# soedinglab/MMseqs2

Measured on AMD Instinct MI355X. Metric: sw_gcells_per_s, higher is better.
Workload: dtype int16

## Files before the change

mmseqs2_amd/csrc/mmgpu_internal.h:

```cpp
#ifndef MMGPU_INTERNAL_H
#define MMGPU_INTERNAL_H

#include <hip/hip_runtime.h>
#include <stdint.h>
#include <cstdlib>
#include <cstring>

#include <algorithm>
#include <array>
#include <string>
#include <map>
#include <mutex>
#include <chrono>
#include <memory>
#include <vector>
#include <thread>
#include <atomic>

#include "../../include/mmgpu.h"
#include "nucl_core.h"
#include "block_plan.h"

namespace mmgpu {

struct DeviceDb {
    uint8_t *res = nullptr;
    uint32_t *off4 = nullptr;
    uint32_t *len = nullptr;
    uint32_t n = 0;
    uint32_t max_len = 0;
    uint64_t total_residues = 0;
    int alphabet = 0;
    size_t res_bytes = 0;
};

struct TargetView {
    const uint8_t *res = nullptr;
    const uint32_t *off4 = nullptr;
    const uint32_t *len = nullptr;
    uint32_t n = 0;
    uint32_t max_len = 0;
    const uint32_t *h_len = nullptr;
};

struct SwMaskGatherArgs {
    const uint8_t *src_res;
    const uint32_t *src_off4, *src_len;
    const uint32_t *src_id;
    uint8_t *dst_res;
    const uint32_t *dst_off4;
    const uint32_t *span_off;
    const mmgpu_sw_span *spans;
    uint32_t span_base;
    uint32_t mask_letter;
    uint32_t n_pairs;
};
hipError_t launch_sw_mask_gather(const SwMaskGatherArgs &A, hipStream_t stream);

struct SwJob {
    uint32_t query;
    uint32_t hit_begin;
    uint32_t hit_end;
    uint32_t shape;
};

struct SwLaunch {
    const SwJob *jobs;
    uint32_t n_jobs;
    const uint8_t *q_res;
    const int8_t *q_cb;
    const uint32_t *q_off;
    const int32_t *q_bias;
    const int32_t *q_minstart;
    const int8_t *q_prof;
    const uint32_t *q_prof_off;
    const uint8_t *t_res;
    const uint32_t *t_off4;
    const uint32_t *t_len;
    const uint32_t *hit_target;
    const uint32_t *hit_out;
    mmgpu_sw_hit *out;
    const int8_t *mat;
    int alphabet;
    int gap_open, gap_extend;
    uint2 *scratch;
    uint32_t scratch_cols;
    uint32_t *scratch_busy;
    uint32_t scratch_slots;
    uint32_t resident_lds = 0;
    const uint32_t *q_hit_count;
    uint32_t hit_stride;
    int rev_mode = 0;
    int rev_only = 0;
    const uint8_t *rev_force = nullptr;
};

constexpr int SW_PF_MAX_LIST = 16384;
constexpr int SW_FROM_PF_STAT_SLOTS = 64;

struct SwFromPfArgs {
    const mmgpu_pf_hit *pf_hits;
    uint32_t pf_stride;
    const uint32_t *hit_count;
    uint32_t stride;
    const uint32_t *q_off;
    const uint32_t *t_len;
    uint32_t *hit_target, *hit_out;
    unsigned long long *cells, *pairs;
    uint32_t *count_copy;
    uint32_t *slot_target;
};

constexpr int SW_REV_JOB_MAX = 1024;
hipError_t launch_sw_rev_multi(const SwLaunch &L, size_t lds_bytes, hipStream_t stream);
hipError_t launch_sw_from_pf(const SwFromPfArgs &A, uint32_t nq, hipStream_t stream);
uint32_t sw_multi_resident_blocks(size_t lds_bytes, bool both_passes, int compute_units);

#ifndef MMGPU_SW_MAX_R
#define MMGPU_SW_MAX_R 28
#endif
constexpr int SW_MAX_R = MMGPU_SW_MAX_R;
static_assert(SW_MAX_R >= 16 && SW_MAX_R <= 32, "multi-tile bodies exist for 8..32 rows per lane: a query cut into tiles gets at least SW_MAX_R / 2");
#ifndef MMGPU_SW_MIN_WAVES
#define MMGPU_SW_MIN_WAVES 2
#endif
constexpr int SW_MIN_WAVES = MMGPU_SW_MIN_WAVES;
#ifndef MMGPU_SW_GROUPS
#define MMGPU_SW_GROUPS 4
#endif
constexpr int SW_GROUPS = MMGPU_SW_GROUPS;
static_assert(SW_GROUPS == 3 || SW_GROUPS == 4, "three or four kernel groups");
int sw_shape_group(uint32_t shape);
hipError_t launch_sw(const SwLaunch &L, int group, size_t lds_bytes, bool both_passes, hipStream_t stream);

constexpr int SW_LDS_HEADER = SW_REV_JOB_MAX * 2 + 64;
__host__ __device__ constexpr int lane_stride_bytes(int R) {
    int slots = (R * 2 + 15) / 16;
    if ((slots & 1) == 0) slots += 1;
    return slots * 16;
}
__host__ __device__ constexpr uint32_t sw_profile_bytes(int R, int alphabet) {
    return (uint32_t)(alphabet + 1) * 16u * (uint32_t)lane_stride_bytes(R);
}
#ifndef MMGPU_SW_RESIDENT_LDS
#define MMGPU_SW_RESIDENT_LDS 65536
#endif
constexpr uint32_t SW_RESIDENT_LDS = MMGPU_SW_RESIDENT_LDS;
static_assert(SW_RESIDENT_LDS <= 65536u, "a workgroup asks for at most 64 KB of dynamic LDS");
__host__ __device__ constexpr uint32_t sw_tiles(uint32_t qlen, int R) { return (qlen + 16u * (uint32_t)R - 1u) / (16u * (uint32_t)R); }
__host__ __device__ constexpr bool sw_multi_resident(uint32_t n_tiles, int R, int alphabet, uint32_t budget) {
    return (unsigned long long)n_tiles * sw_profile_bytes(R, alphabet) + (unsigned long long)SW_LDS_HEADER <= (unsigned long long)budget;
}
static_assert(sw_multi_resident(2, 28, 21, 65536) && sw_multi_resident(3, 24, 21, 65536) && !sw_multi_resident(3, 25, 21, 65536) &&
              !sw_multi_resident(4, 22, 21, 65536) && !sw_multi_resident(2, 8, 21, 0), "residency rule");

constexpr int SCAN_CLASSES = 5;
constexpr int SCAN_MULTI = SCAN_CLASSES - 1;
constexpr int SCAN_MAX_R = 32;
constexpr int SCAN_ROUND = 32;
constexpr int SCAN_JOB_TARGETS = 16 * SCAN_ROUND;
constexpr int SCAN_MAX_HITS = 4096;
__host__ __device__ constexpr int scan_class_rows(int cls) { return cls == 0 ? 8 : cls == 1 ? 16 : cls == 2 ? 24 : 32; }
__host__ __device__ constexpr uint32_t scan_cols(uint32_t len, int R) { return (len + (uint32_t)R - 1u) / (uint32_t)R * (uint32_t)R; }
__host__ __device__ constexpr uint32_t scan_park_row_words(uint32_t longest) { return 2u * ((scan_cols(longest, SCAN_MAX_R) + 1u + 15u) & ~15u); }

constexpr uint64_t SCAN_NO_PROFILE = ~0ull;

struct ScanJob {
    uint32_t query;
    uint32_t begin, end;
    uint32_t pad;
};

struct ScanLaunch {
    const ScanJob *jobs;
    uint32_t n_jobs;
    const uint8_t *q_res;
    const int8_t *q_cb;
    const uint32_t *q_off;
    const int32_t *q_cap;
    const int8_t *q_prof;
    const uint64_t *q_prof_off;
    const uint32_t *q_prof_letters;
    const uint8_t *t_res;
    const uint32_t *t_off4, *t_len;
    const uint32_t *order;
    uint32_t n_targets;
    const int8_t *mat;
    int alphabet;
    uint8_t *scores;
    uint32_t *park;
    const uint64_t *park_off;
};
hipError_t launch_scan(const ScanLaunch &L, int cls, uint32_t grid, hipStream_t stream);

struct ScanSelectArgs {
    const uint8_t *scores;
    const uint32_t *t_len;
    uint32_t n_targets;
    const uint32_t *q_ident;
    const uint32_t *q_win;
    int32_t min_score;
    uint32_t max_hits;
    mmgpu_pf_hit *hits;
    uint32_t stride;
    uint32_t *counts;
};
hipError_t launch_scan_select(const ScanSelectArgs &A, uint32_t nq, hipStream_t stream);
void warm_scan();

constexpr int PF_T = 4096;
constexpr int PF_IDS_PER_BIN = 4096;
constexpr int PF_SAT_CAP = 1024;
constexpr int PF_CAND0 = 32;
constexpr int PF_QSTAGE = 2048;
constexpr int PF_MAX_HITS = 4096;
constexpr int PF_MAX_HITS_BIG = 131072;

struct PfList {
    uint32_t start;
    uint32_t len;
    uint32_t lprefix;
    uint32_t pos;
};

struct PfCand {
    uint32_t id;
    uint32_t arr;
    uint32_t score;
    uint16_t diag;
    uint16_t pad;
};

__host__ __device__ inline uint32_t pf_el_count(uint32_t s) { return (s & 0x80000000u) ? ((s >> 23) & 0xFFu) : (s < 255u ? s : 255u); }
__host__ __device__ inline uint32_t pf_el_exact(uint32_t s) { return (s & 0x80000000u) ? (s & 0x7FFFFFu) : s; }

constexpr int PF_PROW = 32;
constexpr int PF_PROF_LETTERS = 20;

struct PfKmerArgs {
    const uint8_t *q_res;
    const int16_t *q_thr;
    uint32_t n_pos;
    uint8_t pat[16];
    uint32_t kalph, n3;
    uint32_t kbase;
    const int16_t *s3;
    const uint32_t *i3;
    const uint32_t *offsets;
    const uint32_t *nonempty;
    const uint4 *cofs;
    const uint16_t *cum3;
    uint32_t cum_w;
    int32_t score_min;
    int k;
    const int16_t *s2;
    const uint32_t *i2;
    const uint16_t *cum2;
    uint32_t cum2_w;
    int32_t score2_min;
    const uint8_t *q_kind;
    const int16_t *prof_score;
    const uint8_t *prof_letter;
    int exact;
    const uint32_t *order;
    uint32_t *nsim;
    const uint32_t *list_base;
    PfList *lists;
    uint32_t *pos_entries;
};

struct PfSplitArgs {
    const uint32_t *tile_q, *tile_idx;
    const uint32_t *q_off;
    const uint32_t *q_entries;
    const uint32_t *pos_entry_base;
    const uint32_t *list_base;
    const PfList *lists;
    const uint64_t *idx_entries;
    uint32_t bins;
    uint32_t *split;
    uint8_t *split_hi;
    uint16_t *bin_off;
    uint32_t *bucket_count;
};

struct PfDedupArgs {
    uint32_t n_queries, bins;
    uint32_t q_first;
    uint32_t cand_origin;
    const uint32_t *q_tile_base, *q_ntiles;
    const uint32_t *split;
    const uint8_t *split_hi;
    const uint16_t *bin_off;
    const uint32_t *cand_base;
    PfCand *cand, *surv;
    PfCand *cand_small;
    uint32_t *surv_count;
    uint32_t *cand_count;
    uint64_t *cell_counter;
    const uint32_t *q_off;
    const uint8_t *q_res;
    const int8_t *q_corr;
    const int8_t *mat;
    int alphabet;
    const int8_t *q_rows;
    const uint8_t *q_isprof;
    int nucl;
    uint32_t sort_cap;
    uint32_t *q_ncand;
    PfCand *sat;
    uint32_t *q_nsat;
    uint32_t sat_cap;
    const uint8_t *t_res;
    const uint32_t *t_off4, *t_len;
    uint32_t min_diag_score;
    uint32_t *q_flags;
    uint32_t ref_bins;
    uint32_t *big_list, *big_count;
    const uint32_t *q_nseg;
    const uint32_t *seg_start;
};

struct PfSelectArgs {
    uint32_t q_first, cand_origin;
    int kmer_score;
    const PfCand *surv;
    const uint32_t *cand_base;
    uint32_t bins;
    const uint32_t *surv_count;
    const uint32_t *q_identity;
    const int32_t *q_self_score;
    uint32_t max_hits, min_diag_score, ref_bins;
    mmgpu_pf_hit *hits;
    uint32_t hit_stride;
    uint32_t *hit_count, *q_diag_thr;
    mmgpu_pf_xhit *xhits;
    const uint32_t *global_ids;
    const uint32_t *q_nseg;
    uint32_t *q_flags;
    const uint32_t *cand_count;
    uint32_t cand_cap;
    int nucl;
    uint64_t *big_keys;
    uint16_t *big_diags;
    uint32_t big_stride;
    const uint32_t *q_off, *peb, *list_base;
    const PfList *lists;
};

constexpr int PF_XMERGE_CAP = 4096;
struct PfXMergeArgs {
    const mmgpu_pf_xhit *xhits;
    const uint32_t *counts;
    uint32_t n_shards, nq, stride;
    uint32_t max_hits, min_diag_score, ref_bins;
    const int32_t *q_self_score;
    const uint32_t *q_identity;
    mmgpu_pf_hit *out_hits;
    uint32_t out_stride;
    uint32_t *out_counts;
    uint32_t *out_flags;
};
hipError_t launch_pf_xmerge(const PfXMergeArgs &A, hipStream_t s);

struct PfLocalizeArgs {
    const mmgpu_pf_hit *hits;
    const uint32_t *counts;
    uint32_t nq, stride, shard;
    const uint32_t *shard_of, *local_id;
    mmgpu_pf_hit *local_hits;
    uint32_t *local_counts;
    uint32_t *local_slot;
};
hipError_t launch_pf_localize(const PfLocalizeArgs &A, hipStream_t s);

struct SwOwnedRec {
    mmgpu_sw_hit hit;
    uint32_t slot;
    uint32_t pad;
};
struct SwOwnedPackArgs {
    const mmgpu_sw_hit *res;
    const uint32_t *local_counts;
    const uint32_t *local_slot;
    uint32_t nq, stride;
    SwOwnedRec *send;
    uint32_t cap;
    uint32_t *counter;
};
struct SwOwnedScatterArgs {
    const SwOwnedRec *recv;
    const uint32_t *counters;
    uint32_t n_ranks, cap, n_slots;
    mmgpu_sw_hit *full;
    uint32_t *status;
};
hipError_t launch_sw_owned_pack(const SwOwnedPackArgs &A, hipStream_t s);
hipError_t launch_sw_owned_scatter(const SwOwnedScatterArgs &A, hipStream_t s);

constexpr int PF_MAX_SEG = 62;

struct PfSegArgs {
    const uint32_t *ovf_queries;
    uint32_t n_ovf;
    const uint32_t *q_off, *list_base, *pos_entry_base;
    const PfList *lists;
    uint64_t cap;
    uint32_t *seg_start;
    uint32_t *q_nseg;
    uint32_t *q_final;
    const uint32_t *q_entries;
};

struct PfOvfElem {
    uint32_t id;
    uint32_t score;
    long long ord;
    uint16_t diag;
    uint16_t pad0;
    uint32_t pad1;
};

struct PfOvfArgs {
    PfDedupArgs D;
    const uint32_t *ovf_queries;
    uint32_t n_ovf;
    uint32_t step;
    const uint32_t *q_final;
    const uint64_t *ovf_base;
    PfOvfElem *buf_a, *buf_b;
    uint32_t *o_count;
    uint32_t *totals;
};

hipError_t launch_pf_segments(const PfSegArgs &A, hipStream_t s);
hipError_t launch_pf_overflow(const PfOvfArgs &A, hipStream_t s);

constexpr int PF_MERGE_CAP = 8192;

struct PfMergeArgs {
    const mmgpu_pf_hit *hits;
    const uint32_t *counts;
    uint32_t n_splits, nq, stride;
    uint32_t id_offset[64];
    mmgpu_pf_hit *out_hits;
    uint32_t *out_counts;
};

hipError_t launch_pf_merge(const PfMergeArgs &A, hipStream_t s);
hipError_t launch_pf_kmers(const PfKmerArgs &A, bool emit, hipStream_t s);
size_t pf_cofs_bytes(uint64_t table);
hipError_t launch_pf_cofs(const uint32_t *offsets, uint64_t table, void *cofs, hipStream_t s);
hipError_t db_section_checksum(const void *dev, size_t bytes, unsigned long long *scratch, uint64_t *sum, hipStream_t s);
hipError_t db_validate_layout(const uint32_t *off4, const uint32_t *len, uint32_t n, uint64_t res_bytes, uint32_t max_len, const uint32_t *offsets,
                              uint64_t table, const uint64_t *entries, uint64_t n_entries, uint32_t *scratch, uint32_t *bad, hipStream_t s);
hipError_t launch_pf_tiles(const uint32_t *q_tile_base, const uint32_t *q_ntiles, uint32_t nq, uint32_t *tile_q, uint32_t *tile_idx, hipStream_t s);
hipError_t launch_pf_bitmap(const uint32_t *offsets, uint64_t table, uint32_t *bitmap, unsigned long long *nonempty, hipStream_t s);
hipError_t launch_pf_scan(const uint32_t *in, const uint32_t *q_off, uint32_t nq, const uint64_t *base, uint32_t *out,
                          uint64_t *totals, hipStream_t s);
hipError_t launch_pf_split(const PfSplitArgs &A, uint32_t n_tiles, hipStream_t s);
hipError_t launch_pf_dedup(const PfDedupArgs &A, hipEvent_t after_replay, hipEvent_t after_ungapped, hipStream_t s);
hipError_t launch_pf_count(const PfDedupArgs &A, hipEvent_t after_a, hipEvent_t after_b, hipStream_t s);
hipError_t launch_pf_long(const PfDedupArgs &A, bool long_queries, hipStream_t s);
hipError_t launch_pf_select(const PfSelectArgs &A, uint32_t nq, hipStream_t s);

struct IxArgs {
    const uint8_t *t_res;
    const uint32_t *t_off4, *t_len;
    uint32_t n_targets;
    int k, pattern_len, kmer_thr;
    uint32_t kalph;
    uint8_t pat[16];
    int8_t self_score[32];
    uint32_t *counts;
    const uint32_t *offsets;
    uint64_t *entries;
    uint32_t *scratch;
};

struct IxSortArgs {
    uint64_t table;
    const uint32_t *offsets;
    const uint64_t *src;
    uint64_t *dst;
    uint32_t *long_lists;
    uint32_t *n_long;
    uint32_t long_cap;
};

hipError_t launch_ix_target(const IxArgs &A, bool fill, hipStream_t s);

struct TantanArgs {
    const uint8_t *t_res;
    uint8_t *out_res;
    const uint32_t *t_off4, *t_len;
    const uint32_t *order;
    uint32_t n;
    const double *lr;
    const double *b2f;
    int alphabet;
    double repeat_prob, repeat_end_prob, min_mask_prob;
    uint8_t mask_letter;
    float *probs;
    double *scales;
    const uint64_t *wave_prob_base, *wave_scale_base;
    unsigned long long *n_masked;
};
hipError_t launch_tantan_mask(const TantanArgs &A, hipStream_t s);
void warm_sw();
void warm_block();
void warm_pf();
void warm_ix();
void warm_tantan();
void warm_bt();
hipError_t launch_ix_sort_short(const IxSortArgs &A, hipStream_t s);
hipError_t launch_ix_sort_long(const IxSortArgs &A, uint32_t n_long, hipStream_t s);

struct BtJob {
    uint32_t slot;
    uint32_t query, target;
    int32_t q_start, q_end, t_start, t_end, score;
    uint64_t bt_off;
};

struct BtLaunch {
    const BtJob *jobs;
    uint32_t n_jobs;
    const uint8_t *q_res;
    const int8_t *q_cb;
    const uint32_t *q_off;
    const int8_t *q_prof;
    const uint32_t *q_prof_off;
    const uint8_t *t_res;
    const uint32_t *t_off4;
    const int8_t *mat;
    int alphabet, gap_open, gap_extend;
    uint32_t *scratch;
    uint32_t words_per_lane;
    uint32_t band_cap;
    mmgpu_sw_bt *info;
    char *bt;
    uint8_t *dir_pool;
    unsigned long long dir_pool_bytes;
    unsigned long long *dir_cursor;
};

struct BlockLaunch {
    const BlockJob *jobs;
    uint32_t n_jobs;
    const uint8_t *q_res;
    const int8_t *q_cb;
    const uint32_t *q_off;
    const uint8_t *t_res;
    const uint32_t *t_off4;
    const int8_t *q_prof;
    const uint32_t *q_prof_off;
    int alphabet;
    const int8_t *scores;
    int gap_open, gap_extend;
    mmgpu_sw_block *out;
    const uint64_t *bt_off;
    char *bt;
    uint8_t *pool;
    uint64_t slot_bytes;
    uint32_t n_pool_slots;
    uint32_t *pool_busy;
    uint32_t *growth = nullptr;
    uint32_t growth_cap = 0;
};
hipError_t launch_sw_block(const BlockLaunch &L, int tier, hipStream_t stream);

struct Block2Launch {
    const Block2Job *jobs;
    uint32_t n_jobs;
    uint32_t *counter;
    const uint8_t *q_res;
    const int8_t *q_cb;
    const uint32_t *q_off;
    const uint8_t *t_res;
    const uint32_t *t_off4;
    const int8_t *scores;
    int gap_open, gap_extend;
    mmgpu_sw_block *out;
    const uint64_t *bt_off;
    char *bt;
    uint8_t *pool;
    uint32_t *growth = nullptr;
    uint32_t growth_cap = 0;
    uint8_t *ck_pool = nullptr;
    uint32_t trace_bytes = 0;
};
constexpr int BLOCK4_MAX_SIZE = 128;
constexpr int BLOCK4_LARGE_SIZE = 256;
constexpr int BLOCK4_SKEW_SIZE = 1024;
hipError_t launch_sw_block4(const Block2Launch &L, bool trace, int form, uint32_t n_waves, hipStream_t stream);
hipError_t launch_sw_block4_walk(const Block2Launch &L, hipStream_t stream);
void warm_block4();

struct BlockSelectArgs {
    const mmgpu_sw_hit *res;
    uint32_t pairs;
    const uint32_t *qout_off;
    uint32_t n_queries;
    const int32_t *q_minstart;
    const uint32_t *slot_target;
    BlockJob *jobs;
    uint32_t *pair_of_slot;
    mmgpu_sw_block *blk;
    uint32_t *count;
    uint32_t cap;
};
struct BlockScatterArgs {
    const mmgpu_sw_block *blk;
    const uint32_t *pair_of_slot;
    uint32_t n;
    mmgpu_sw_hit *res;
    uint8_t *rev_force;
    uint32_t *counts;
};
hipError_t launch_block_select(const BlockSelectArgs &A, hipStream_t stream);
hipError_t launch_block_scatter(const BlockScatterArgs &A, hipStream_t stream);

hipError_t launch_sw_traceback(const BtLaunch &L, hipStream_t stream);
hipError_t launch_sw_traceback_wave(const BtLaunch &L, hipStream_t stream);

inline unsigned host_threads() {
    unsigned n = std::thread::hardware_concurrency();
    return n == 0 ? 1 : std::min(n, 64u);
}

template <typename F>
inline void parallel_for(size_t n, F f) {
    const unsigned nt = (unsigned)std::min<size_t>(host_threads(), std::max<size_t>(n, 1));
    if (nt <= 1 || n < 4096) {
        f((size_t)0, n);
        return;
    }
    std::vector<std::thread> th;
    const size_t chunk = (n + nt - 1) / nt;
    for (unsigned t = 0; t < nt; t++) {
        const size_t a = std::min(n, (size_t)t * chunk), b = std::min(n, a + chunk);
        if (a < b) th.emplace_back([=] { f(a, b); });
    }
    for (auto &x : th) x.join();
}

extern thread_local std::string g_last_error;
inline int fail(int code, const std::string &msg) {
    g_last_error = msg;
    return code;
}
#define HIP_TRY(expr)                                                                                      \
    do {                                                                                                   \
        hipError_t e__ = (expr);                                                                           \
        if (e__ != hipSuccess)                                                                             \
            return mmgpu::fail(MMGPU_ERR_HIP, std::string(#expr) + ": " + hipGetErrorString(e__));         \
    } while (0)

inline hipError_t dev_malloc(void **p, size_t n) { return hipMalloc(p, n); }
inline void dev_free(void *p) {
    if (p) (void)hipFree(p);
}

struct BlockCache {
    std::multimap<size_t, void *> blocks;
    size_t cached = 0;
    bool closed = false;
    std::mutex lock;
    static size_t limit() {
        static const size_t v = []() -> size_t {
            size_t f = 0, t = 0;
            if (hipMemGetInfo(&f, &t) != hipSuccess || t == 0) return (size_t)16 << 30;
            return t / 3;
        }();
        return v;
    }
    static size_t round_up(size_t n) {
        if (n <= 512) return 512;
        int top = 63 - __builtin_clzll((unsigned long long)n);
        const size_t step = (size_t)1 << (top - 2);
        return (n + step - 1) & ~(step - 1);
    }
    void *take(size_t &cap) {
        std::lock_guard<std::mutex> guard(lock);
        auto it = blocks.lower_bound(cap);
        if (it == blocks.end() || it->first > 2 * cap) return nullptr;
        void *p = it->second;
        cap = it->first;
        blocks.erase(it);
        cached -= cap;
        return p;
    }
    void give(void *p, size_t cap) {
        std::lock_guard<std::mutex> guard(lock);
        if (closed || cached + cap > limit()) { dev_free(p); return; }
        blocks.emplace(cap, p);
        cached += cap;
    }
    void trim() {
        std::lock_guard<std::mutex> guard(lock);
        for (auto &kv : blocks) dev_free(kv.second);
        blocks.clear();
        cached = 0;
    }
};

struct DevBuf {
    void *p = nullptr;
    size_t bytes = 0;
    size_t cap = 0;
    std::shared_ptr<BlockCache> cache;
    DevBuf() = default;
    DevBuf(const DevBuf &) = delete;
    DevBuf &operator=(const DevBuf &) = delete;
    DevBuf(DevBuf &&o) noexcept : p(o.p), bytes(o.bytes), cap(o.cap), cache(std::move(o.cache)) { o.p = nullptr; o.bytes = 0; o.cap = 0; }
    DevBuf &operator=(DevBuf &&o) noexcept {
        if (this != &o) {
            release();
            p = o.p; bytes = o.bytes; cap = o.cap; cache = std::move(o.cache);
            o.p = nullptr; o.bytes = 0; o.cap = 0;
        }
        return *this;
    }
    ~DevBuf() { release(); }
    void bind(const std::shared_ptr<BlockCache> &c) {
        cache = c;
    }
    void release() {
        if (!p) return;
        if (cache && cap) cache->give(p, cap);
        else dev_free(p);
        p = nullptr;
        cap = 0;
    }
    hipError_t alloc(size_t n) {
        release();
        bytes = n;
        if (n == 0) return hipSuccess;
        if (cache) {
            cap = BlockCache::round_up(n);
            p = cache->take(cap);
            if (p) return hipSuccess;
            hipError_t e = dev_malloc(&p, cap);
            if (e != hipSuccess) {
                (void)hipGetLastError();
                cache->trim();
                e = dev_malloc(&p, cap);
            }
            if (e != hipSuccess) { p = nullptr; cap = 0; bytes = 0; }
            return e;
        }
        const hipError_t e = dev_malloc(&p, n);
        if (e != hipSuccess) { p = nullptr; bytes = 0; (void)hipGetLastError(); }
        return e;
    }
    hipError_t reserve(size_t n) { return n <= bytes ? hipSuccess : alloc(n + n / 8); }
    template <typename T> T *as() const { return reinterpret_cast<T *>(p); }
};

struct SideStream {
    hipStream_t s = nullptr;
    SideStream() = default;
    SideStream(const SideStream &) = delete;
    SideStream &operator=(const SideStream &) = delete;
    ~SideStream() { if (s) { (void)hipStreamSynchronize(s); (void)hipStreamDestroy(s); } }
    hipError_t create() { return s ? hipSuccess : hipStreamCreateWithFlags(&s, hipStreamNonBlocking); }
};

struct PinnedStage {
    uint8_t *p = nullptr;
    hipEvent_t moved = nullptr;
    PinnedStage() = default;
    PinnedStage(const PinnedStage &) = delete;
    PinnedStage &operator=(const PinnedStage &) = delete;
    ~PinnedStage() { if (p) (void)hipHostFree(p); if (moved) (void)hipEventDestroy(moved); }
    hipError_t reserve(size_t bytes, bool with_event = true) {
        const hipError_t e = hipHostMalloc((void **)&p, bytes, hipHostMallocDefault);
        if (e != hipSuccess) { p = nullptr; return e; }
        return with_event ? hipEventCreateWithFlags(&moved, hipEventDisableTiming) : hipSuccess;
    }
};

struct UploadRing {
    SideStream up;
    std::vector<PinnedStage> slots;
    UploadRing() = default;
    UploadRing(const UploadRing &) = delete;
    UploadRing &operator=(const UploadRing &) = delete;
    ~UploadRing() { if (up.s) (void)hipStreamSynchronize(up.s); }
    hipError_t open(size_t n_slots) { slots = std::vector<PinnedStage>(n_slots); return up.create(); }
    hipError_t wait(size_t k) const { return hipEventSynchronize(slots[k].moved); }
    hipError_t sent(size_t k) const { return hipEventRecord(slots[k].moved, up.s); }
};

struct DbBuild {
    DeviceDb db;
    uint8_t *masked = nullptr;
    DbBuild() = default;
    DbBuild(const DbBuild &) = delete;
    DbBuild &operator=(const DbBuild &) = delete;
    ~DbBuild() { dev_free(db.res); dev_free(db.off4); dev_free(db.len); dev_free(masked); }
    DeviceDb take_db() { DeviceDb d = db; db = DeviceDb(); return d; }
    uint8_t *take_masked() { uint8_t *m = masked; masked = nullptr; return m; }
};

template <typename T>
inline hipError_t upload(DevBuf &b, const std::vector<T> &v, hipStream_t s) {
    hipError_t e = b.alloc(std::max<size_t>(v.size(), 1) * sizeof(T));
    if (e != hipSuccess) return e;
    if (v.empty()) return hipSuccess;
    return hipMemcpyAsync(b.p, v.data(), v.size() * sizeof(T), hipMemcpyHostToDevice, s);
}

inline size_t upload_pinned_need(size_t bytes) { return (bytes + 255) & ~(size_t)255; }
template <typename T>
inline hipError_t upload_pinned(DevBuf &b, const std::vector<T> &v, hipStream_t s, void *base, size_t cap, size_t &used) {
    hipError_t e = b.alloc(std::max<size_t>(v.size(), 1) * sizeof(T));
    if (e != hipSuccess) return e;
    if (v.empty()) return hipSuccess;
    const size_t n = v.size() * sizeof(T);
    if (!base || used + upload_pinned_need(n) > cap) return hipMemcpyAsync(b.p, v.data(), n, hipMemcpyHostToDevice, s);
    void *st = static_cast<char *>(base) + used;
    used += upload_pinned_need(n);
    memcpy(st, v.data(), n);
    return hipMemcpyAsync(b.p, st, n, hipMemcpyHostToDevice, s);
}

hipError_t launch_nucl_align(const NuclLaunch &L, unsigned blocks, hipStream_t stream);
hipError_t launch_nucl_align_wave(const NuclLaunch &L, unsigned blocks, hipStream_t stream);

hipError_t launch_pf_order(const PfKmerArgs &A, uint32_t *order, const std::shared_ptr<BlockCache> &cache, hipStream_t s);

struct PfIndex;

}

namespace mmgpu {
struct Comm {
    void *nccl = nullptr;
    int rank = 0, n_ranks = 1;
    std::string transport;
};
}

struct mmgpu_ctx {
    int device = 0;
    mmgpu::Comm *comm = nullptr;
    hipStream_t stream = nullptr;
    bool owns_stream = false;
    mmgpu::DeviceDb db;
    std::vector<uint32_t> h_len;
    uint32_t mean_len = 0;
    int compute_units = 0;
    std::string name;
    mmgpu::PfIndex *pf = nullptr;
    uint8_t *pf_masked_res = nullptr;
    const uint8_t *pf_res() const { return pf_masked_res ? pf_masked_res : db.res; }
    struct Shard {
        bool on = false;
        uint32_t n_shards = 1, shard = 0, global_n = 0;
        mmgpu::DevBuf d_global_ids, d_shard_of, d_local_id;
    } shard;
    std::shared_ptr<mmgpu::BlockCache> cache = std::make_shared<mmgpu::BlockCache>();
    hipStream_t side[4] = {};
    hipEvent_t fork = nullptr, join[4] = {};
    void *pinned = nullptr;
    size_t pinned_cap = 0;
    std::atomic<bool> pinned_busy{false};
    mmgpu::DevBuf scan_scores, scan_park;
    uint64_t scan_serial = 0;
};

inline hipError_t dev_malloc_ctx(mmgpu_ctx *c, void **p, size_t n) {
    hipError_t e = mmgpu::dev_malloc(p, n);
    if (e != hipSuccess && c && c->cache) {
        (void)hipGetLastError();
        c->cache->trim();
        e = mmgpu::dev_malloc(p, n);
    }
    return e;
}

struct mmgpu_pf_batch_t;
struct mmgpu_sw_batch_t;
namespace mmgpu {
int comm_require_rccl();
int comm_group_start();
int comm_group_end();
int comm_init_all(mmgpu_ctx **ctxs, int n);
int comm_allgather(mmgpu_ctx *c, const void *send, void *recv, size_t bytes);
void comm_free(mmgpu_ctx *c);
struct XchgBlock { const void *send; void *recv; size_t bytes; };
int pf_xchg_begin(mmgpu_ctx *c, mmgpu_pf_batch_t *b, int n_ranks, XchgBlock blocks[2]);
int pf_xchg_merge(mmgpu_ctx *c, mmgpu_pf_batch_t *b, int n_ranks, const uint32_t *identity_global);
struct PfRedoRows {
    std::vector<uint32_t> q;
    std::vector<mmgpu_pf_hit> hits;
    std::vector<uint32_t> counts;
    std::vector<int32_t> status;
    uint32_t stride = 0;
};
int pf_redo_flagged(mmgpu_ctx *c, mmgpu_pf_batch_t *b, std::vector<uint32_t> &flagged);
int pf_redo_run(mmgpu_ctx *full, const mmgpu_pf_params *par, const mmgpu_pf_query *qs, const std::vector<uint32_t> &flagged, PfRedoRows &rows);
int pf_redo_apply(mmgpu_ctx *c, mmgpu_pf_batch_t *b, const PfRedoRows &rows);
const int32_t *pf_batch_redo_status(const mmgpu_pf_batch_t *b);
int sw_gather_begin(mmgpu_ctx *c, mmgpu_sw_batch_t *b, int n_ranks, XchgBlock blocks[2]);
int sw_gather_finish(mmgpu_ctx *c, mmgpu_sw_batch_t *b, int n_ranks);
int sw_gather_overflowed(mmgpu_ctx *c, mmgpu_sw_batch_t *b, bool *overflowed);
int pf_batch_merged_flags(mmgpu_pf_batch_t *b, const void **d_flags);
const int32_t *pf_batch_host_status(const mmgpu_pf_batch_t *b);
bool pf_batch_merged_lists(mmgpu_pf_batch_t *b, const mmgpu_pf_hit **hits, const uint32_t **counts, uint32_t *stride, uint32_t *nq);
void pf_index_free(mmgpu_ctx *c);
void db_release(mmgpu_ctx *c);
bool pf_batch_device_lists(mmgpu_pf_batch_t *b, const mmgpu_pf_hit **hits, const uint32_t **counts, uint32_t *stride, uint32_t *nq);
}
#endif
```

mmseqs2_amd/csrc/sw_kernel.hip:

```cpp
#include "mmgpu_internal.h"
#include "pf_device.h"

namespace mmgpu {

namespace {

constexpr int GROUP = 16;
constexpr int WAVES = 4;
constexpr int GROUPS_PER_WAVE = 64 / GROUP;
constexpr int HITS_PER_WAVE = 2 * GROUPS_PER_WAVE;
constexpr unsigned NEG2 = 0x80008000u;

typedef short s16x2 __attribute__((ext_vector_type(2)));
typedef unsigned short u16x2 __attribute__((ext_vector_type(2)));

__device__ __forceinline__ unsigned pk_add_sat(unsigned a, unsigned b) {
    return __builtin_bit_cast(unsigned, __builtin_elementwise_add_sat(__builtin_bit_cast(s16x2, a),
                                                                      __builtin_bit_cast(s16x2, b)));
}
__device__ __forceinline__ unsigned pk_max_s(unsigned a, unsigned b) {
    return __builtin_bit_cast(unsigned, __builtin_elementwise_max(__builtin_bit_cast(s16x2, a),
                                                                  __builtin_bit_cast(s16x2, b)));
}
__device__ __forceinline__ unsigned pk_max_u(unsigned a, unsigned b) {
    return __builtin_bit_cast(unsigned, __builtin_elementwise_max(__builtin_bit_cast(u16x2, a),
                                                                  __builtin_bit_cast(u16x2, b)));
}
__device__ __forceinline__ unsigned pk_sub_sat_u(unsigned a, unsigned b) {
    return __builtin_bit_cast(unsigned, __builtin_elementwise_sub_sat(__builtin_bit_cast(u16x2, a),
                                                                      __builtin_bit_cast(u16x2, b)));
}
__device__ __forceinline__ unsigned bfi(unsigned mask, unsigned a, unsigned b) {
    return (a & mask) | (b & ~mask);
}
__device__ __forceinline__ unsigned from_lane_above(unsigned head, unsigned v) {
    return __builtin_amdgcn_update_dpp(head, v, 0x111 , 0xF, 0xF, false);
}
__device__ __forceinline__ unsigned from_lane_above_or_zero(unsigned v) {
    return __builtin_amdgcn_update_dpp(0u, v, 0x111 , 0xF, 0xF, true);
}

#ifndef MMGPU_SW_PREFETCH
#define MMGPU_SW_PREFETCH 1
#endif
#define SW_KEEP_IN_ROW(x) asm volatile("" : "+v"(x))

template <int R>
struct Tile {
    static constexpr int ROWS = GROUP * R;
    static constexpr int LANE_STRIDE = lane_stride_bytes(R);
    static constexpr int ROW_STRIDE = GROUP * LANE_STRIDE;
};
static_assert(GROUP == 16, "sw_profile_bytes and sw_tiles (mmgpu_internal.h) assume 16-lane groups");

template <int R, bool REV>
__device__ __forceinline__ void build_profile(unsigned char *lds, const uint8_t *q, const int8_t *cb, int qlen,
                                              int tile_base, const int8_t *mat, int alphabet, const int8_t *prof) {
    using T = Tile<R>;
    const int total = (alphabet + 1) * T::ROWS;
    for (int idx = threadIdx.x; idx < total; idx += blockDim.x) {
        const int letter = idx / T::ROWS;
        const int row = idx - letter * T::ROWS;
        const int rg = tile_base + row;
        short v = (short)-32768;
        if (letter < alphabet && rg < qlen) {
            const int qi = REV ? (qlen - 1 - rg) : rg;
            v = prof ? (short)prof[letter * qlen + qi] : (short)((int)mat[letter * alphabet + q[qi]] + (int)cb[qi]);
        }
        const int lane = row / R, r = row - lane * R;
        *reinterpret_cast<short *>(lds + letter * T::ROW_STRIDE + lane * T::LANE_STRIDE + r * 2) = v;
    }
}

__device__ __forceinline__ bool sw_rev_wanted(const SwLaunch &L, uint32_t slot, int min_start) {
    const mmgpu_sw_hit &f = L.out[slot];
    const int s = f.score;
    if (L.rev_mode == 2) return s > 0 && L.rev_force[slot] != 0;
    return s > 0 && s >= min_start && !(L.rev_mode == 1 && f.word != 0);
}

constexpr int SW_REV_JOB_HITS = 1024;
static_assert(SW_REV_JOB_HITS == SW_REV_JOB_MAX, "host and kernel disagree on the reverse job size");
static_assert(SW_LDS_HEADER == SW_REV_JOB_HITS * 2 + 64, "the header holds the live hits and the scheduling words");

template <int R, bool MULTI, bool REV, bool PF>
__device__ __forceinline__ void sw_body(const SwLaunch &L, const SwJob job) {
    using T = Tile<R>;
    extern __shared__ __attribute__((aligned(16))) unsigned char lds_all[];
    uint16_t *live = reinterpret_cast<uint16_t *>(lds_all);
    uint32_t *live_wave = reinterpret_cast<uint32_t *>(lds_all + SW_REV_JOB_HITS * 2);
    uint32_t *next_chunk = reinterpret_cast<uint32_t *>(lds_all + SW_REV_JOB_HITS * 2 + 16);
    unsigned char *lds = lds_all + SW_LDS_HEADER;
    if (MULTI) __builtin_amdgcn_s_setprio(3);
    const int lane = threadIdx.x & 63;
    const int wave = __builtin_amdgcn_readfirstlane(threadIdx.x >> 6);
    const int g = lane & (GROUP - 1);
    const int grp = lane / GROUP;

    const uint32_t qbeg = L.q_off[job.query];
    const int qlen = (int)(L.q_off[job.query + 1] - qbeg);
    const uint8_t *q = L.q_res + qbeg;
    const int8_t *cb = L.q_cb + qbeg;
    const int qbias = L.q_bias[job.query];
    const int8_t *prof = nullptr;
    if (L.q_prof_off) {
        const uint32_t po = L.q_prof_off[job.query];
        if (po != 0xFFFFFFFFu) prof = L.q_prof + po;
    }
    const int n_tiles = MULTI ? (int)sw_tiles((uint32_t)qlen, R) : 1;
    const uint32_t tile_bytes = sw_profile_bytes(R, L.alphabet);
    const bool resident = MULTI && sw_multi_resident((uint32_t)n_tiles, R, L.alphabet, L.resident_lds);
    const bool dynamic = !MULTI || resident;
    auto build_all_tiles = [&]() {
        for (int tile = 0; tile < n_tiles; ++tile)
            build_profile<R, REV>(lds + (uint32_t)tile * tile_bytes, q, cb, qlen, tile * T::ROWS, L.mat, L.alphabet, prof);
        __syncthreads();
    };

    const unsigned go2 = (unsigned)L.gap_open * 0x10001u;
    const unsigned ge2 = (unsigned)L.gap_extend * 0x10001u;
    const unsigned pad_letter = (unsigned)L.alphabet;

    if (threadIdx.x == 0) *next_chunk = 0;
    if (!MULTI && !REV) {
        build_profile<R, REV>(lds, q, cb, qlen, 0, L.mat, L.alphabet, prof);
        __syncthreads();
    }
    if (MULTI && !REV && resident) build_all_tiles();

    uint32_t n_hits = job.hit_end - job.hit_begin;
    if (REV) {
        const int min_start = L.q_minstart[job.query];
        uint32_t total = 0;
        for (uint32_t base = 0; base < n_hits; base += WAVES * 64) {
            const uint32_t idx = base + threadIdx.x;
            bool pass = false;
            if (idx < n_hits) pass = sw_rev_wanted(L, L.hit_out[job.hit_begin + idx], min_start);
            const unsigned long long bal = __ballot(pass);
            if (lane == 0) live_wave[wave] = (uint32_t)__popcll(bal);
            __syncthreads();
            uint32_t before = 0, round_total = 0;
#pragma unroll
            for (int w = 0; w < WAVES; ++w) {
                const uint32_t c = live_wave[w];
                before += w < wave ? c : 0u;
                round_total += c;
            }
            if (pass) live[total + before + (uint32_t)__popcll(bal & ((1ull << lane) - 1ull))] = (uint16_t)idx;
            total += round_total;
            __syncthreads();
        }
        n_hits = total;
        if (n_hits == 0) return;
        if (!MULTI) {
            build_profile<R, REV>(lds, q, cb, qlen, 0, L.mat, L.alphabet, prof);
            __syncthreads();
        }
        if (MULTI && resident) build_all_tiles();
    }
    const uint32_t n_iter = (n_hits + WAVES * HITS_PER_WAVE - 1) / (WAVES * HITS_PER_WAVE);

    for (uint32_t it = 0; dynamic || it < n_iter; ++it) {
        uint32_t chunk = it * WAVES + wave;
        if (dynamic) {
            if (lane == 0) chunk = atomicAdd(next_chunk, 1u);
            chunk = __builtin_amdgcn_readfirstlane(chunk);
        }
        const uint32_t slot0 = chunk * HITS_PER_WAVE;
        if (dynamic && slot0 >= n_hits) break;

        const uint32_t sA = slot0 + grp * 2, sB = sA + 1;
        const bool vA = sA < n_hits, vB = sB < n_hits;
        const uint32_t hA = job.hit_begin + (REV ? (uint32_t)live[vA ? sA : 0] : sA);
        const uint32_t hB = job.hit_begin + (REV ? (uint32_t)live[vB ? sB : 0] : sB);
        const uint32_t tA = vA ? L.hit_target[hA] : 0u, tB = vB ? L.hit_target[hB] : 0u;
        const uint8_t *pA = L.t_res + (size_t)L.t_off4[tA] * 4;
        const uint8_t *pB = L.t_res + (size_t)L.t_off4[tB] * 4;
        int colsA = vA ? (int)L.t_len[tA] : 0, colsB = vB ? (int)L.t_len[tB] : 0;
        int r0A = 0, r0B = 0;
        int endA = 0, endB = 0;
        unsigned rev_target = 0xFFFFFFFFu;
        if (REV) {
            mmgpu_sw_hit fa, fb;
            fa.score = 0; fa.q_end = 0; fa.t_end = 0;
            fb = fa;
            if (vA) fa = L.out[L.hit_out[hA]];
            if (vB) fb = L.out[L.hit_out[hB]];
            colsA = vA ? fa.t_end + 1 : 0;
            colsB = vB ? fb.t_end + 1 : 0;
            endA = colsA > 0 ? fa.t_end : 0;
            endB = colsB > 0 ? fb.t_end : 0;
            r0A = colsA > 0 ? qlen - 1 - fa.q_end : 0;
            r0B = colsB > 0 ? qlen - 1 - fb.q_end : 0;
            rev_target = (colsA > 0 ? (unsigned)fa.score & 0xFFFFu : 0xFFFFu) | ((colsB > 0 ? (unsigned)fb.score & 0xFFFFu : 0xFFFFu) << 16);
        }
        int ncols = colsA > colsB ? colsA : colsB;
        ncols = max(ncols, __shfl_xor(ncols, 16));
        ncols = max(ncols, __shfl_xor(ncols, 32));
        ncols = __builtin_amdgcn_readfirstlane(ncols);
        const int nsteps = ncols + GROUP - 1;
        int mincols = colsA < colsB ? colsA : colsB;
        mincols = min(mincols, __shfl_xor(mincols, 16));
        mincols = min(mincols, __shfl_xor(mincols, 32));
        mincols = __builtin_amdgcn_readfirstlane(mincols);

        unsigned long long bestA = 0, bestB = 0;

        uint2 *scr = nullptr;
        unsigned scr_grp = 0;
        if (MULTI) {
            scr = L.scratch + (size_t)((job.shape >> 8) * WAVES + wave) * GROUPS_PER_WAVE * 2 * L.scratch_cols;
            scr_grp = (unsigned)grp * 2u * L.scratch_cols;
        }

        for (int tile = 0; tile < n_tiles; ++tile) {
            const int tile_base = tile * T::ROWS;
            if (MULTI && !resident) {
                __syncthreads();
                build_profile<R, REV>(lds, q, cb, qlen, tile_base, L.mat, L.alphabet, prof);
                __syncthreads();
            }
            const unsigned char *const lds_tile = MULTI && resident ? lds + (uint32_t)tile * tile_bytes : lds;
            const uint2 *scr_in = MULTI ? scr + (size_t)((tile + 1) & 1) * L.scratch_cols : nullptr;
            uint2 *scr_out = MULTI ? scr + (size_t)(tile & 1) * L.scratch_cols : nullptr;
            const bool has_above = MULTI && tile > 0;
            const bool has_below = MULTI && tile + 1 < n_tiles;

            unsigned Hp[R], E[R], aux[R];
#pragma unroll
            for (int r = 0; r < R; ++r) { Hp[r] = 0; E[r] = 0; aux[r] = 0; }
            if (REV) {
#pragma unroll
                for (int r = 0; r < R; ++r) {
                    const int rg = tile_base + g * R + r;
                    aux[r] = (rg >= r0A ? 0xFFFFu : 0u) | (rg >= r0B ? 0xFFFF0000u : 0u);
                }
            }
            unsigned vmax = 0, bestcol = 0xFFFFFFFFu;
            unsigned rev_rowA = 0, rev_rowB = 0;
            unsigned Hup_prev = 0;
            unsigned out_H = 0, out_F = 0;

            auto letters4 = [&](const uint8_t *p, int end, int k) -> unsigned {
                if (!REV) return reinterpret_cast<const unsigned *>(p)[k];
                int o = end - 3 - 4 * k;
                o = o < -3 ? -3 : o;
                unsigned w;
                __builtin_memcpy(&w, p + o, 4);
                return w;
            };
            unsigned wA = letters4(pA, endA, 0), wB = letters4(pB, endB, 0);
            unsigned wA_next = letters4(pA, endA, 1), wB_next = letters4(pB, endB, 1);
            uint2 bnd = make_uint2(0, 0), bnd_next = make_uint2(0, 0);
            auto boundary16 = [&](int m) -> uint2 {
                const int last = ncols - 1 < 0 ? 0 : ncols - 1;
                return scr_in[scr_grp + (unsigned)min(16 * m + g - (m > 0 ? 1 : 0), last)];
            };
            if (has_above) {
                bnd = boundary16(0);
                bnd_next = boundary16(1);
            }

            constexpr int ND = (R + 1) / 2;
            unsigned pav_next[PF ? ND : 1], pbv_next[PF ? ND : 1];
            auto load_rows = [&](unsigned letters, unsigned *pav, unsigned *pbv) {
                const unsigned a = letters & 0xFFu, b = (letters >> 8) & 0xFFu;
                const uint4 *rowA = reinterpret_cast<const uint4 *>(lds_tile + a * T::ROW_STRIDE + g * T::LANE_STRIDE);
                const uint4 *rowB = reinterpret_cast<const uint4 *>(lds_tile + b * T::ROW_STRIDE + g * T::LANE_STRIDE);
#pragma unroll
                for (int k = 0; k < ND / 4; ++k) {
                    const uint4 pa = rowA[k], pb = rowB[k];
                    pav[4 * k] = pa.x; pav[4 * k + 1] = pa.y; pav[4 * k + 2] = pa.z; pav[4 * k + 3] = pa.w;
                    pbv[4 * k] = pb.x; pbv[4 * k + 1] = pb.y; pbv[4 * k + 2] = pb.z; pbv[4 * k + 3] = pb.w;
                }
                if constexpr (ND % 4 >= 2) {
                    const uint2 pa = *reinterpret_cast<const uint2 *>(rowA + ND / 4);
                    const uint2 pb = *reinterpret_cast<const uint2 *>(rowB + ND / 4);
                    pav[(ND / 4) * 4] = pa.x; pav[(ND / 4) * 4 + 1] = pa.y;
                    pbv[(ND / 4) * 4] = pb.x; pbv[(ND / 4) * 4 + 1] = pb.y;
                }
                if constexpr (ND % 2 == 1) {
                    pav[ND - 1] = reinterpret_cast<const unsigned *>(rowA)[ND - 1];
                    pbv[ND - 1] = reinterpret_cast<const unsigned *>(rowB)[ND - 1];
                }
            };
            unsigned let = pad_letter * 0x101u;
            constexpr bool LETTER_BLOCKS = MULTI || REV || R >= 7;
            constexpr bool LETTER_QUEUE = !MULTI && R < 7;
            unsigned long long lq = 0;
            auto letter_block = [&](int k) {
                if (!LETTER_BLOCKS) return;
                unsigned a = wA, b = wB;
                if (4 * k + 4 > mincols) {
                    const unsigned pad4 = pad_letter * 0x01010101u;
                    const int na = min(max(colsA - 4 * k, 0), 4), nb = min(max(colsB - 4 * k, 0), 4);
                    const unsigned ma = REV ? ~(unsigned)(0xFFFFFFFFull >> (8 * na)) : (unsigned)((1ull << (8 * na)) - 1ull);
                    const unsigned mb = REV ? ~(unsigned)(0xFFFFFFFFull >> (8 * nb)) : (unsigned)((1ull << (8 * nb)) - 1ull);
                    a = bfi(ma, a, pad4);
                    b = bfi(mb, b, pad4);
                }
                const unsigned lo = __builtin_amdgcn_perm(b, a, REV ? 0x06020703u : 0x05010400u);
                const unsigned hi = __builtin_amdgcn_perm(b, a, REV ? 0x04000501u : 0x07030602u);
                lq = ((unsigned long long)hi << 32) | lo;
            };
            auto head_letters = [&](int c, int j) -> unsigned {
                if (LETTER_BLOCKS && LETTER_QUEUE) { const unsigned v = (unsigned)lq; lq >>= 16; return v; }
                if (LETTER_BLOCKS) return (unsigned)(lq >> (16 * j));
                const unsigned sh = (unsigned)(REV ? 3 - j : j) * 8u;
                const unsigned la0 = __builtin_amdgcn_ubfe(wA, sh, 8u);
                const unsigned lb0 = __builtin_amdgcn_ubfe(wB, sh, 8u);
                return (c < colsA ? la0 : pad_letter) | ((c < colsB ? lb0 : pad_letter) << 8);
            };
            letter_block(0);
            let = from_lane_above(head_letters(0, 0), let);
            if (PF) load_rows(let, pav_next, pbv_next);

            for (int s0 = -1; s0 < nsteps; s0 += 4) {
            if (MULTI && s0 > 0 && ((s0 + 1) & 15) == 0) {
                bnd = bnd_next;
                if (has_above) bnd_next = boundary16(((s0 + 1) >> 4) + 1);
            }
            const int jn = min(4, nsteps - s0);
#pragma nounroll
            for (int j = s0 < 0 ? 1 : 0; j < jn; ++j) {
                const int s = s0 + j;
                if (has_below && s >= GROUP) {
                    if (g == GROUP - 1) (scr_out + (s - GROUP))[scr_grp] = make_uint2(out_H, out_F);
                }
                const unsigned Hup = MULTI ? from_lane_above(bnd.x, out_H) : from_lane_above_or_zero(out_H);
                unsigned f = MULTI ? from_lane_above(bnd.y, out_F) : from_lane_above_or_zero(out_F);
                if (MULTI) {
                    bnd.x = __builtin_amdgcn_update_dpp(bnd.x, bnd.x, 0x12F, 0xF, 0xF, false);
                    bnd.y = __builtin_amdgcn_update_dpp(bnd.y, bnd.y, 0x12F, 0xF, 0xF, false);
                }
                unsigned pav[ND], pbv[ND];
                if (PF) {
#pragma unroll
                    for (int k = 0; k < ND; ++k) { pav[k] = pav_next[k]; pbv[k] = pbv_next[k]; }
                } else {
                    load_rows(let, pav, pbv);
                }

                unsigned hd = Hup_prev;
                Hup_prev = Hup;
                unsigned cmax = 0;
                unsigned pre[R], es[R];
#pragma unroll
                for (int r = 0; r < R; ++r) {
                    unsigned P = __builtin_amdgcn_perm(pbv[r / 2], pav[r / 2], (r & 1) ? 0x07060302u : 0x05040100u);
                    if (REV) P = __builtin_amdgcn_bitop3_b32(aux[r], P, NEG2, 0xCA);
                    pre[r] = pk_max_s(pk_add_sat(r == 0 ? hd : Hp[r - 1], P), E[r]);
                    es[r] = pk_sub_sat_u(E[r], ge2);
                }
                let = from_lane_above(head_letters(s + 1, j), let);
                if (PF) load_rows(let, pav_next, pbv_next);
#pragma unroll
                for (int r = 0; r < R; ++r) {
                    const unsigned h = pk_max_s(pre[r], f);
                    const unsigned fs = pk_sub_sat_u(f, ge2);
                    const unsigned t = pk_sub_sat_u(h, go2);
                    cmax = pk_max_u(cmax, h);
                    f = pk_max_u(fs, t);
                    E[r] = pk_max_u(es[r], t);
                    SW_KEEP_IN_ROW(E[r]);
                    Hp[r] = h;
                }
                out_H = Hp[R - 1];
                out_F = f;

                const int col = s - g;

                const unsigned nm = pk_max_u(vmax, cmax);
                if (nm != vmax) {
                    const unsigned diff = nm ^ vmax;
                    if (!REV) {
                        const unsigned mask = ((diff & 0xFFFFu) ? 0xFFFFu : 0u) | ((diff >> 16) ? 0xFFFF0000u : 0u);
                        bestcol = bfi(mask, ((unsigned)col & 0xFFFFu) * 0x10001u, bestcol);
#pragma unroll
                        for (int r = 0; r < R; ++r) aux[r] = bfi(mask, Hp[r], aux[r]);
                    } else {
                        const unsigned x = nm ^ rev_target;
                        const bool hitA = (diff & 0xFFFFu) && !(x & 0xFFFFu), hitB = (diff >> 16) && !(x >> 16);
                        if (hitA | hitB) {
                            asm volatile("" ::: "memory");
                            unsigned ra = 0, rb = 0;
#pragma unroll
                            for (int r = R - 1; r >= 0; --r) {
                                if ((Hp[r] & 0xFFFFu) == (rev_target & 0xFFFFu)) ra = (unsigned)r;
                                if ((Hp[r] >> 16) == (rev_target >> 16)) rb = (unsigned)r;
                            }
                            if (hitA) { bestcol = (bestcol & 0xFFFF0000u) | ((unsigned)col & 0xFFFFu); rev_rowA = ra; }
                            if (hitB) { bestcol = (bestcol & 0xFFFFu) | ((unsigned)col << 16); rev_rowB = rb; }
                        }
                    }
                    vmax = nm;
                }
            }
            {
                wA = wA_next; wB = wB_next;
                const int k = ((s0 + 1) >> 2) + 2;
                wA_next = letters4(pA, endA, k); wB_next = letters4(pB, endB, k);
                letter_block(k - 1);
            }
            }
            if (has_below && ncols > 0 && g == GROUP - 1) (scr_out + (ncols - 1))[scr_grp] = make_uint2(out_H, out_F);

            unsigned rowA_first = rev_rowA, rowB_first = rev_rowB;
            unsigned sA = vmax & 0xFFFFu, sB = vmax >> 16;
            if (!REV) {
#pragma unroll
                for (int r = R - 1; r >= 0; --r) {
                    if ((aux[r] & 0xFFFFu) == sA) rowA_first = (unsigned)r;
                    if ((aux[r] >> 16) == sB) rowB_first = (unsigned)r;
                }
            } else {
                sA = sA == (rev_target & 0xFFFFu) ? sA : 0u;
                sB = sB == (rev_target >> 16) ? sB : 0u;
            }
            const unsigned rgA = (unsigned)(tile_base + g * R) + rowA_first;
            const unsigned rgB = (unsigned)(tile_base + g * R) + rowB_first;
            unsigned long long keyA = sA ? ((unsigned long long)sA << 32) | ((0xFFFFu - (bestcol & 0xFFFFu)) << 16) | (0xFFFFu - rgA) : 0ull;
            unsigned long long keyB = sB ? ((unsigned long long)sB << 32) | ((0xFFFFu - (bestcol >> 16)) << 16) | (0xFFFFu - rgB) : 0ull;
#pragma unroll
            for (int m = 1; m < GROUP; m <<= 1) {
                const unsigned long long oa = __shfl_xor(keyA, m), ob = __shfl_xor(keyB, m);
                keyA = oa > keyA ? oa : keyA;
                keyB = ob > keyB ? ob : keyB;
            }
            bestA = keyA > bestA ? keyA : bestA;
            bestB = keyB > bestB ? keyB : bestB;
        }

        if (g == 0) {
#pragma unroll
            for (int half = 0; half < 2; ++half) {
                const bool valid = half ? vB : vA;
                if (!valid) continue;
                const unsigned long long key = half ? bestB : bestA;
                const uint32_t h = half ? hB : hA;
                const int score = (int)(key >> 32);
                const int col = 0xFFFF - (int)((key >> 16) & 0xFFFFu);
                const int row = 0xFFFF - (int)(key & 0xFFFFu);
                mmgpu_sw_hit *o = L.out + L.hit_out[h];
                if (!REV) {
                    mmgpu_sw_hit res;
                    res.score = score;
                    res.q_end = score ? row : 0;
                    res.t_end = score ? col : -1;
                    res.q_start = -1;
                    res.t_start = -1;
                    res.word = (score + qbias >= 255) ? 1 : 0;
                    *o = res;
                } else {
                    const int end = half ? endB : endA;
                    const int cols = half ? colsB : colsA;
                    if (cols > 0) {
                        o->t_start = (score == o->score) ? end - col : -2;
                        o->q_start = (score == o->score) ? qlen - 1 - row : -2;
                    }
                }
            }
        }
    }
}

template <int R, bool MULTI, bool BOTH>
__device__ __forceinline__ void sw_passes(const SwLaunch &L, const SwJob &job) {
    if constexpr (R <= SW_MAX_R) {
        constexpr bool PF = MMGPU_SW_PREFETCH && !MULTI && (BOTH || R <= 24);
        if (!(BOTH && L.rev_only)) sw_body<R, MULTI, false, PF>(L, job);
        if constexpr (BOTH && !MULTI) {
            __threadfence_block();
            __syncthreads();
            sw_body<R, MULTI, true, PF>(L, job);
        }
    }
}

#ifndef MMGPU_SW_WAVES_G0F
#define MMGPU_SW_WAVES_G0F 4
#endif
#ifndef MMGPU_SW_WAVES_G0B
#define MMGPU_SW_WAVES_G0B 2
#endif
#ifndef MMGPU_SW_WAVES_G1F
#define MMGPU_SW_WAVES_G1F 3
#endif
#ifndef MMGPU_SW_WAVES_G1B
#define MMGPU_SW_WAVES_G1B 2
#endif
#define MMGPU_SW_MULTI_ALL                                                                                                          \
    MMGPU_SW_MULTI(8) MMGPU_SW_MULTI(9) MMGPU_SW_MULTI(10) MMGPU_SW_MULTI(11) MMGPU_SW_MULTI(12) MMGPU_SW_MULTI(13) MMGPU_SW_MULTI(14) \
    MMGPU_SW_MULTI(15) MMGPU_SW_MULTI(16) MMGPU_SW_MULTI(17) MMGPU_SW_MULTI(18) MMGPU_SW_MULTI(19) MMGPU_SW_MULTI(20) MMGPU_SW_MULTI(21) \
    MMGPU_SW_MULTI(22) MMGPU_SW_MULTI(23) MMGPU_SW_MULTI(24) MMGPU_SW_MULTI(25) MMGPU_SW_MULTI(26) MMGPU_SW_MULTI(27) MMGPU_SW_MULTI(28) \
    MMGPU_SW_MULTI(29) MMGPU_SW_MULTI(30) MMGPU_SW_MULTI(31) MMGPU_SW_MULTI(32)
template <int G, bool BOTH>
__global__ __launch_bounds__(WAVES * 64)
__attribute__((amdgpu_waves_per_eu(G == 0 ? (BOTH ? MMGPU_SW_WAVES_G0B : MMGPU_SW_WAVES_G0F)
                                           : (G == 1 ? (BOTH ? MMGPU_SW_WAVES_G1B : MMGPU_SW_WAVES_G1F) : SW_MIN_WAVES),
                                   G == 1 && BOTH ? MMGPU_SW_WAVES_G1B : 8))) void sw_kernel(SwLaunch L) {
    SwJob job = L.jobs[blockIdx.x];
    if (L.q_hit_count) {
        const uint32_t lim = job.query * L.hit_stride + L.q_hit_count[job.query];
        job.hit_end = job.hit_end < lim ? job.hit_end : lim;
        if (job.hit_end <= job.hit_begin) return;
    }
    __shared__ uint32_t scratch_slot;
    const bool claims = G == SW_GROUPS - 1 && (job.shape & 0xFFu) >= 32u;
    if (claims) {
        if (threadIdx.x == 0) {
            uint32_t s = blockIdx.x % L.scratch_slots;
            while (atomicCAS(&L.scratch_busy[s], 0u, 1u) != 0u) s = s + 1 == L.scratch_slots ? 0u : s + 1;
            scratch_slot = s;
        }
        __syncthreads();
        job.shape = (job.shape & 0xFFu) | (scratch_slot << 8);
    }
#define MMGPU_SW_SINGLE(R) case (R) - 1: sw_passes<R, false, BOTH>(L, job); break;
#define MMGPU_SW_MULTI(R) case 32 + (R) - 1: sw_passes<R, true, BOTH>(L, job); break;
    if constexpr (G == 0) {
        switch (job.shape & 0xFFu) {
            MMGPU_SW_SINGLE(1) MMGPU_SW_SINGLE(2) MMGPU_SW_SINGLE(3) MMGPU_SW_SINGLE(4) MMGPU_SW_SINGLE(5) MMGPU_SW_SINGLE(6)
            MMGPU_SW_SINGLE(7) MMGPU_SW_SINGLE(8) MMGPU_SW_SINGLE(9) MMGPU_SW_SINGLE(10) MMGPU_SW_SINGLE(11) MMGPU_SW_SINGLE(12)
            default: break;
        }
    } else if constexpr (G == 1) {
        switch (job.shape & 0xFFu) {
            MMGPU_SW_SINGLE(13) MMGPU_SW_SINGLE(14) MMGPU_SW_SINGLE(15) MMGPU_SW_SINGLE(16) MMGPU_SW_SINGLE(17) MMGPU_SW_SINGLE(18)
            MMGPU_SW_SINGLE(19) MMGPU_SW_SINGLE(20) MMGPU_SW_SINGLE(21) MMGPU_SW_SINGLE(22) MMGPU_SW_SINGLE(23) MMGPU_SW_SINGLE(24)
            default: break;
        }
    } else if constexpr (SW_GROUPS == 4 && G == 2) {
        switch (job.shape & 0xFFu) {
            MMGPU_SW_SINGLE(25) MMGPU_SW_SINGLE(26) MMGPU_SW_SINGLE(27) MMGPU_SW_SINGLE(28) MMGPU_SW_SINGLE(29) MMGPU_SW_SINGLE(30)
            MMGPU_SW_SINGLE(31) MMGPU_SW_SINGLE(32)
            default: break;
        }
    } else if constexpr (SW_GROUPS == 4) {
        switch (job.shape & 0xFFu) {
            MMGPU_SW_MULTI_ALL
            default: break;
        }
    } else {
        switch (job.shape & 0xFFu) {
            MMGPU_SW_SINGLE(25) MMGPU_SW_SINGLE(26) MMGPU_SW_SINGLE(27) MMGPU_SW_SINGLE(28) MMGPU_SW_SINGLE(29) MMGPU_SW_SINGLE(30)
            MMGPU_SW_SINGLE(31) MMGPU_SW_SINGLE(32)
            MMGPU_SW_MULTI_ALL
            default: break;
        }
    }
#undef MMGPU_SW_SINGLE
#undef MMGPU_SW_MULTI
#undef MMGPU_SW_MULTI_ALL
    if (claims) {
        __syncthreads();
        if (threadIdx.x == 0) {
            __threadfence();
            atomicExch(&L.scratch_busy[scratch_slot], 0u);
        }
    }
}

__global__ __launch_bounds__(WAVES * 64) __attribute__((amdgpu_waves_per_eu(SW_MIN_WAVES))) void sw_rev_multi_kernel(SwLaunch L) {
    SwJob job = L.jobs[blockIdx.x];
    if (L.q_hit_count) {
        const uint32_t lim = job.query * L.hit_stride + L.q_hit_count[job.query];
        job.hit_end = job.hit_end < lim ? job.hit_end : lim;
        if (job.hit_end <= job.hit_begin) return;
    }
    __shared__ uint32_t scratch_slot;
    if (threadIdx.x == 0) {
        uint32_t s = blockIdx.x % L.scratch_slots;
        while (atomicCAS(&L.scratch_busy[s], 0u, 1u) != 0u) s = s + 1 == L.scratch_slots ? 0u : s + 1;
        scratch_slot = s;
    }
    __syncthreads();
    job.shape = (job.shape & 0xFFu) | (scratch_slot << 8);
#define MMGPU_SW_REV(R) case 32 + (R) - 1: if constexpr ((R) <= SW_MAX_R) sw_body<R, true, true, false>(L, job); break;
    switch (job.shape & 0xFFu) {
        MMGPU_SW_REV(8) MMGPU_SW_REV(9) MMGPU_SW_REV(10) MMGPU_SW_REV(11) MMGPU_SW_REV(12) MMGPU_SW_REV(13) MMGPU_SW_REV(14) MMGPU_SW_REV(15)
        MMGPU_SW_REV(16) MMGPU_SW_REV(17) MMGPU_SW_REV(18) MMGPU_SW_REV(19) MMGPU_SW_REV(20) MMGPU_SW_REV(21) MMGPU_SW_REV(22) MMGPU_SW_REV(23)
        MMGPU_SW_REV(24) MMGPU_SW_REV(25) MMGPU_SW_REV(26) MMGPU_SW_REV(27) MMGPU_SW_REV(28) MMGPU_SW_REV(29) MMGPU_SW_REV(30) MMGPU_SW_REV(31)
        MMGPU_SW_REV(32)
        default: break;
    }
#undef MMGPU_SW_REV
    __syncthreads();
    if (threadIdx.x == 0) {
        __threadfence();
        atomicExch(&L.scratch_busy[scratch_slot], 0u);
    }
}

__global__ __launch_bounds__(256) void sw_from_pf_kernel(SwFromPfArgs A) {
    extern __shared__ uint32_t key[];
    const uint32_t q = blockIdx.x;
    unsigned long long *const stat = A.cells + (size_t)(blockIdx.x % (uint32_t)SW_FROM_PF_STAT_SLOTS) * 3;
    const uint32_t n = min(A.hit_count[q], A.stride);
    const mmgpu_pf_hit *hits = A.pf_hits + (size_t)q * A.pf_stride;
    uint32_t np2 = 1;
    while (np2 < n) np2 <<= 1;
    unsigned long long cells = 0;
    const uint32_t qlen = A.q_off[q + 1] - A.q_off[q];
    for (uint32_t k = threadIdx.x; k < np2; k += 256) {
        uint32_t v = 0xFFFFFFFFu;
        if (k < n) {
            const uint32_t len = A.t_len[hits[k].id];
            v = ((0xFFFFu - min(len, 0xFFFFu)) << 16) | k;
            cells += (unsigned long long)qlen * len;
        }
        key[k] = v;
    }
    __syncthreads();
    const uint32_t base = q * A.stride;
    if (n <= 512) {
        for (uint32_t i = threadIdx.x; i < n; i += 256) {
            const uint32_t mine = key[i];
            uint32_t r = 0;
            for (uint32_t j = 0; j < n; j++) r += key[j] < mine ? 1u : 0u;
            A.hit_target[base + r] = hits[i].id;
            A.hit_out[base + r] = base + i;
            A.slot_target[base + i] = hits[i].id;
            if (r == 0) atomicMax(stat + 2, (unsigned long long)(0xFFFFu - (mine >> 16)));
        }
    } else {
    block_bitonic_sort<256>(np2, [&](uint32_t i, uint32_t j) { return key[i] > key[j]; }, [&](uint32_t i, uint32_t j) { exchange_at(key, i, j); });
    for (uint32_t r = threadIdx.x; r < n; r += 256) {
        const uint32_t k = key[r] & 0xFFFFu;
        A.hit_target[base + r] = hits[k].id;
        A.hit_out[base + r] = base + k;
        A.slot_target[base + r] = hits[r].id;
    }
    if (threadIdx.x == 0 && n) atomicMax(stat + 2, (unsigned long long)(0xFFFFu - (key[0] >> 16)));
    }
    for (uint32_t r = n + threadIdx.x; r < A.stride; r += 256) {
        A.hit_target[base + r] = 0;
        A.hit_out[base + r] = base + r;
        A.slot_target[base + r] = 0;
    }
    if (threadIdx.x == 0) A.count_copy[q] = n;
    wave_sum_to(stat, cells);
    if (threadIdx.x == 0 && n) atomicAdd(stat + 1, (unsigned long long)n);
}

}

hipError_t launch_sw_from_pf(const SwFromPfArgs &A, uint32_t nq, hipStream_t stream) {
    static_assert((SW_PF_MAX_LIST & (SW_PF_MAX_LIST - 1)) == 0 && (size_t)SW_PF_MAX_LIST * sizeof(uint32_t) <= 65536,
                  "SW_PF_MAX_LIST: a power of two whose dwords fit 64 KB of dynamic LDS");
    if (A.stride > (uint32_t)SW_PF_MAX_LIST) return hipErrorInvalidValue;
    if (nq == 0) return hipSuccess;
    uint32_t np2 = 1;
    while (np2 < A.stride) np2 <<= 1;
    const size_t lds = (size_t)np2 * sizeof(uint32_t);
    if (lds > 65536) return hipErrorInvalidValue;
    const hipError_t attr = hipFuncSetAttribute(reinterpret_cast<const void *>(sw_from_pf_kernel),
                                                hipFuncAttributeMaxDynamicSharedMemorySize, 65536);
    if (attr != hipSuccess) return attr;
    hipLaunchKernelGGL(sw_from_pf_kernel, dim3(nq), dim3(256), lds, stream, A);
    return hipGetLastError();
}

uint32_t sw_multi_resident_blocks(size_t lds_bytes, bool both_passes, int compute_units) {
    int per_cu = 0;
    const size_t lds = lds_bytes + SW_LDS_HEADER;
    hipError_t e = both_passes ? hipOccupancyMaxActiveBlocksPerMultiprocessor(&per_cu, sw_kernel<SW_GROUPS - 1, true>, WAVES * 64, lds)
                               : hipOccupancyMaxActiveBlocksPerMultiprocessor(&per_cu, sw_kernel<SW_GROUPS - 1, false>, WAVES * 64, lds);
    if (e == hipSuccess && both_passes) {
        int rev = 0;
        if (hipOccupancyMaxActiveBlocksPerMultiprocessor(&rev, sw_rev_multi_kernel, WAVES * 64, lds) == hipSuccess) per_cu = std::max(per_cu, rev);
    }
    if (e != hipSuccess || per_cu < 1) per_cu = 8;
    per_cu = per_cu + 1 > 8 ? 8 : per_cu + 1;
    return (uint32_t)per_cu * (uint32_t)(compute_units > 0 ? compute_units : 256);
}

hipError_t launch_sw_rev_multi(const SwLaunch &L, size_t lds_bytes, hipStream_t stream) {
    if (L.n_jobs == 0) return hipSuccess;
    hipLaunchKernelGGL(sw_rev_multi_kernel, dim3(L.n_jobs), dim3(WAVES * 64), lds_bytes + SW_LDS_HEADER, stream, L);
    return hipGetLastError();
}

int sw_shape_group(uint32_t shape) {
    if (shape >= 32) return SW_GROUPS - 1;
    const int R = (int)shape + 1;
    return R <= 12 ? 0 : (R <= 24 ? 1 : 2);
}

hipError_t launch_sw(const SwLaunch &L, int group, size_t lds_bytes, bool both_passes, hipStream_t stream) {
    static_assert(GROUP == 16, "the shape codes assume 16-lane groups");
    if (L.n_jobs == 0) return hipSuccess;
    dim3 grid(L.n_jobs), block(WAVES * 64);
    const size_t lds = lds_bytes + SW_LDS_HEADER;
    switch (group * 2 + (both_passes ? 1 : 0)) {
        case 0: hipLaunchKernelGGL((sw_kernel<0, false>), grid, block, lds, stream, L); break;
        case 1: hipLaunchKernelGGL((sw_kernel<0, true>), grid, block, lds, stream, L); break;
        case 2: hipLaunchKernelGGL((sw_kernel<1, false>), grid, block, lds, stream, L); break;
        case 3: hipLaunchKernelGGL((sw_kernel<1, true>), grid, block, lds, stream, L); break;
        case 4: hipLaunchKernelGGL((sw_kernel<2, false>), grid, block, lds, stream, L); break;
        case 5: hipLaunchKernelGGL((sw_kernel<2, true>), grid, block, lds, stream, L); break;
        case 6: hipLaunchKernelGGL((sw_kernel<SW_GROUPS - 1, false>), grid, block, lds, stream, L); break;
        case 7: hipLaunchKernelGGL((sw_kernel<SW_GROUPS - 1, true>), grid, block, lds, stream, L); break;
        default: return hipErrorInvalidValue;
    }
    return hipGetLastError();
}

void warm_sw() {
    hipFuncAttributes a;
    (void)hipFuncGetAttributes(&a, reinterpret_cast<const void *>(&sw_rev_multi_kernel));
}

}
```

Baseline: 4674.

## Add f16 packed Smith-Waterman path with int16 re-run for saturated hits

```diff
diff --git a/mmseqs2_amd/csrc/mmgpu_internal.h b/mmseqs2_amd/csrc/mmgpu_internal.h
--- a/mmseqs2_amd/csrc/mmgpu_internal.h
+++ b/mmseqs2_amd/csrc/mmgpu_internal.h
@@ -132,6 +132,11 @@
 static_assert(SW_GROUPS == 3 || SW_GROUPS == 4, "three or four kernel groups");
 int sw_shape_group(uint32_t shape);
 hipError_t launch_sw(const SwLaunch &L, int group, size_t lds_bytes, bool both_passes, hipStream_t stream);
+#ifndef MMGPU_SW_HALF
+#define MMGPU_SW_HALF 1
+#endif
+bool launch_sw_half(const SwLaunch &L, int group, size_t lds_bytes, bool both_passes, hipStream_t stream);
+void warm_sw_half();
 
 constexpr int SW_LDS_HEADER = SW_REV_JOB_MAX * 2 + 64;
 __host__ __device__ constexpr int lane_stride_bytes(int R) {
diff --git a/mmseqs2_amd/csrc/sw_body.h b/mmseqs2_amd/csrc/sw_body.h
--- /dev/null
+++ b/mmseqs2_amd/csrc/sw_body.h
@@ -0,0 +1,543 @@
+#pragma once
+#include "mmgpu_internal.h"
+#include "pf_device.h"
+
+namespace mmgpu {
+
+namespace {
+
+constexpr int GROUP = 16;
+constexpr int WAVES = 4;
+constexpr int GROUPS_PER_WAVE = 64 / GROUP;
+constexpr int HITS_PER_WAVE = 2 * GROUPS_PER_WAVE;
+constexpr unsigned NEG2 = 0x80008000u;
+
+typedef short s16x2 __attribute__((ext_vector_type(2)));
+typedef unsigned short u16x2 __attribute__((ext_vector_type(2)));
+
+__device__ __forceinline__ unsigned pk_add_sat(unsigned a, unsigned b) {
+    return __builtin_bit_cast(unsigned, __builtin_elementwise_add_sat(__builtin_bit_cast(s16x2, a),
+                                                                      __builtin_bit_cast(s16x2, b)));
+}
+__device__ __forceinline__ unsigned pk_max_s(unsigned a, unsigned b) {
+    return __builtin_bit_cast(unsigned, __builtin_elementwise_max(__builtin_bit_cast(s16x2, a),
+                                                                  __builtin_bit_cast(s16x2, b)));
+}
+__device__ __forceinline__ unsigned pk_max_u(unsigned a, unsigned b) {
+    return __builtin_bit_cast(unsigned, __builtin_elementwise_max(__builtin_bit_cast(u16x2, a),
+                                                                  __builtin_bit_cast(u16x2, b)));
+}
+__device__ __forceinline__ unsigned pk_sub_sat_u(unsigned a, unsigned b) {
+    return __builtin_bit_cast(unsigned, __builtin_elementwise_sub_sat(__builtin_bit_cast(u16x2, a),
+                                                                      __builtin_bit_cast(u16x2, b)));
+}
+__device__ __forceinline__ unsigned bfi(unsigned mask, unsigned a, unsigned b) {
+    return (a & mask) | (b & ~mask);
+}
+
+constexpr int SW_HALF_LIMIT = 2048 - 256;
+constexpr int SW_HALF_MAX_GAP = 2048;
+constexpr int SW_HALF_MARK = -1;
+typedef _Float16 h16x2 __attribute__((ext_vector_type(2)));
+__device__ __forceinline__ h16x2 as_h(unsigned a) { return __builtin_bit_cast(h16x2, a); }
+__device__ __forceinline__ unsigned as_u(h16x2 a) { return __builtin_bit_cast(unsigned, a); }
+__device__ __forceinline__ unsigned h_add(unsigned a, unsigned b) { return as_u(as_h(a) + as_h(b)); }
+__device__ __forceinline__ unsigned h_sub(unsigned a, unsigned b) { return as_u(as_h(a) - as_h(b)); }
+__device__ __forceinline__ unsigned h_max(unsigned a, unsigned b) {
+    return as_u(__builtin_elementwise_maximum(as_h(a), as_h(b)));
+}
+__device__ __forceinline__ unsigned h_max3(unsigned a, unsigned b, unsigned c) {
+    return as_u(__builtin_elementwise_maximum(__builtin_elementwise_maximum(as_h(a), as_h(b)), as_h(c)));
+}
+__device__ __forceinline__ unsigned short h_bits(int v) { return __builtin_bit_cast(unsigned short, (_Float16)v); }
+__device__ __forceinline__ int h_value(unsigned bits) { return (int)(float)__builtin_bit_cast(_Float16, (unsigned short)bits); }
+__device__ __forceinline__ unsigned from_lane_above(unsigned head, unsigned v) {
+    return __builtin_amdgcn_update_dpp(head, v, 0x111 , 0xF, 0xF, false);
+}
+__device__ __forceinline__ unsigned from_lane_above_or_zero(unsigned v) {
+    return __builtin_amdgcn_update_dpp(0u, v, 0x111 , 0xF, 0xF, true);
+}
+
+#ifndef MMGPU_SW_PREFETCH
+#define MMGPU_SW_PREFETCH 1
+#endif
+#define SW_KEEP_IN_ROW(x) asm volatile("" : "+v"(x))
+
+template <int R>
+struct Tile {
+    static constexpr int ROWS = GROUP * R;
+    static constexpr int LANE_STRIDE = lane_stride_bytes(R);
+    static constexpr int ROW_STRIDE = GROUP * LANE_STRIDE;
+};
+static_assert(GROUP == 16, "sw_profile_bytes and sw_tiles (mmgpu_internal.h) assume 16-lane groups");
+
+template <int R, bool REV, bool HALF = false>
+__device__ __forceinline__ void build_profile(unsigned char *lds, const uint8_t *q, const int8_t *cb, int qlen,
+                                              int tile_base, const int8_t *mat, int alphabet, const int8_t *prof) {
+    using T = Tile<R>;
+    const int total = (alphabet + 1) * T::ROWS;
+    for (int idx = threadIdx.x; idx < total; idx += blockDim.x) {
+        const int letter = idx / T::ROWS;
+        const int row = idx - letter * T::ROWS;
+        const int rg = tile_base + row;
+        short v = (short)-32768;
+        if (letter < alphabet && rg < qlen) {
+            const int qi = REV ? (qlen - 1 - rg) : rg;
+            v = prof ? (short)prof[letter * qlen + qi] : (short)((int)mat[letter * alphabet + q[qi]] + (int)cb[qi]);
+        }
+        const int lane = row / R, r = row - lane * R;
+        if constexpr (HALF) v = (short)h_bits(v);
+        *reinterpret_cast<short *>(lds + letter * T::ROW_STRIDE + lane * T::LANE_STRIDE + r * 2) = v;
+    }
+}
+
+__device__ __forceinline__ bool sw_rev_wanted(const SwLaunch &L, uint32_t slot, int min_start) {
+    const mmgpu_sw_hit &f = L.out[slot];
+    const int s = f.score;
+    if (L.rev_mode == 2) return s > 0 && L.rev_force[slot] != 0;
+    return s > 0 && s >= min_start && !(L.rev_mode == 1 && f.word != 0);
+}
+
+constexpr int SW_REV_JOB_HITS = 1024;
+static_assert(SW_REV_JOB_HITS == SW_REV_JOB_MAX, "host and kernel disagree on the reverse job size");
+static_assert(SW_LDS_HEADER == SW_REV_JOB_HITS * 2 + 64, "the header holds the live hits and the scheduling words");
+constexpr int SW_HALF_FLAG_AT = SW_REV_JOB_HITS * 2 + 20;
+__device__ __forceinline__ uint32_t sw_half_any_marked() {
+    extern __shared__ __attribute__((aligned(16))) unsigned char lds_all[];
+    return *reinterpret_cast<const uint32_t *>(lds_all + SW_HALF_FLAG_AT);
+}
+
+template <int R, bool MULTI, bool REV, bool PF, bool HALF = false, bool MARKED = false>
+__device__ __forceinline__ void sw_body(const SwLaunch &L, const SwJob job) {
+    static_assert(!(HALF || MARKED) || (!MULTI && !REV && !(HALF && MARKED)), "f16 and its int16 re-run: single-tile forward scans");
+    constexpr bool PACKED = REV || MARKED;
+    using T = Tile<R>;
+    extern __shared__ __attribute__((aligned(16))) unsigned char lds_all[];
+    uint16_t *live = reinterpret_cast<uint16_t *>(lds_all);
+    uint32_t *live_wave = reinterpret_cast<uint32_t *>(lds_all + SW_REV_JOB_HITS * 2);
+    uint32_t *next_chunk = reinterpret_cast<uint32_t *>(lds_all + SW_REV_JOB_HITS * 2 + 16);
+    uint32_t *half_flag = reinterpret_cast<uint32_t *>(lds_all + SW_HALF_FLAG_AT);
+    unsigned char *lds = lds_all + SW_LDS_HEADER;
+    if (MULTI) __builtin_amdgcn_s_setprio(3);
+    const int lane = threadIdx.x & 63;
+    const int wave = __builtin_amdgcn_readfirstlane(threadIdx.x >> 6);
+    const int g = lane & (GROUP - 1);
+    const int grp = lane / GROUP;
+
+    const uint32_t qbeg = L.q_off[job.query];
+    const int qlen = (int)(L.q_off[job.query + 1] - qbeg);
+    const uint8_t *q = L.q_res + qbeg;
+    const int8_t *cb = L.q_cb + qbeg;
+    const int qbias = L.q_bias[job.query];
+    const int8_t *prof = nullptr;
+    if (L.q_prof_off) {
+        const uint32_t po = L.q_prof_off[job.query];
+        if (po != 0xFFFFFFFFu) prof = L.q_prof + po;
+    }
+    const int n_tiles = MULTI ? (int)sw_tiles((uint32_t)qlen, R) : 1;
+    const uint32_t tile_bytes = sw_profile_bytes(R, L.alphabet);
+    const bool resident = MULTI && sw_multi_resident((uint32_t)n_tiles, R, L.alphabet, L.resident_lds);
+    const bool dynamic = !MULTI || resident;
+    auto build_all_tiles = [&]() {
+        for (int tile = 0; tile < n_tiles; ++tile)
+            build_profile<R, REV>(lds + (uint32_t)tile * tile_bytes, q, cb, qlen, tile * T::ROWS, L.mat, L.alphabet, prof);
+        __syncthreads();
+    };
+
+    const unsigned go2 = (HALF ? (unsigned)h_bits(L.gap_open) : (unsigned)L.gap_open) * 0x10001u;
+    const unsigned ge2 = (HALF ? (unsigned)h_bits(L.gap_extend) : (unsigned)L.gap_extend) * 0x10001u;
+    const unsigned pad_letter = (unsigned)L.alphabet;
+
+    if (threadIdx.x == 0) *next_chunk = 0;
+    if (HALF && threadIdx.x == 0) *half_flag = 0;
+    if (!MULTI && !PACKED) {
+        build_profile<R, REV, HALF>(lds, q, cb, qlen, 0, L.mat, L.alphabet, prof);
+        __syncthreads();
+    }
+    if (MULTI && !REV && resident) build_all_tiles();
+
+    uint32_t n_hits = job.hit_end - job.hit_begin;
+    if (PACKED) {
+        const int min_start = REV ? L.q_minstart[job.query] : 0;
+        uint32_t total = 0;
+        for (uint32_t base = 0; base < n_hits; base += WAVES * 64) {
+            const uint32_t idx = base + threadIdx.x;
+            bool pass = false;
+            if (idx < n_hits) {
+                const uint32_t slot = L.hit_out[job.hit_begin + idx];
+                pass = MARKED ? L.out[slot].score == SW_HALF_MARK : sw_rev_wanted(L, slot, min_start);
+            }
+            const unsigned long long bal = __ballot(pass);
+            if (lane == 0) live_wave[wave] = (uint32_t)__popcll(bal);
+            __syncthreads();
+            uint32_t before = 0, round_total = 0;
+#pragma unroll
+            for (int w = 0; w < WAVES; ++w) {
+                const uint32_t c = live_wave[w];
+                before += w < wave ? c : 0u;
+                round_total += c;
+            }
+            if (pass) live[total + before + (uint32_t)__popcll(bal & ((1ull << lane) - 1ull))] = (uint16_t)idx;
+            total += round_total;
+            __syncthreads();
+        }
+        n_hits = total;
+        if (n_hits == 0) return;
+        if (!MULTI) {
+            build_profile<R, REV>(lds, q, cb, qlen, 0, L.mat, L.alphabet, prof);
+            __syncthreads();
+        }
+        if (MULTI && resident) build_all_tiles();
+    }
+    const uint32_t n_iter = (n_hits + WAVES * HITS_PER_WAVE - 1) / (WAVES * HITS_PER_WAVE);
+
+    for (uint32_t it = 0; dynamic || it < n_iter; ++it) {
+        uint32_t chunk = it * WAVES + wave;
+        if (dynamic) {
+            if (lane == 0) chunk = atomicAdd(next_chunk, 1u);
+            chunk = __builtin_amdgcn_readfirstlane(chunk);
+        }
+        const uint32_t slot0 = chunk * HITS_PER_WAVE;
+        if (dynamic && slot0 >= n_hits) break;
+
+        const uint32_t sA = slot0 + grp * 2, sB = sA + 1;
+        const bool vA = sA < n_hits, vB = sB < n_hits;
+        const uint32_t hA = job.hit_begin + (PACKED ? (uint32_t)live[vA ? sA : 0] : sA);
+        const uint32_t hB = job.hit_begin + (PACKED ? (uint32_t)live[vB ? sB : 0] : sB);
+        const uint32_t tA = vA ? L.hit_target[hA] : 0u, tB = vB ? L.hit_target[hB] : 0u;
+        const uint8_t *pA = L.t_res + (size_t)L.t_off4[tA] * 4;
+        const uint8_t *pB = L.t_res + (size_t)L.t_off4[tB] * 4;
+        int colsA = vA ? (int)L.t_len[tA] : 0, colsB = vB ? (int)L.t_len[tB] : 0;
+        int r0A = 0, r0B = 0;
+        int endA = 0, endB = 0;
+        unsigned rev_target = 0xFFFFFFFFu;
+        if (REV) {
+            mmgpu_sw_hit fa, fb;
+            fa.score = 0; fa.q_end = 0; fa.t_end = 0;
+            fb = fa;
+            if (vA) fa = L.out[L.hit_out[hA]];
+            if (vB) fb = L.out[L.hit_out[hB]];
+            colsA = vA ? fa.t_end + 1 : 0;
+            colsB = vB ? fb.t_end + 1 : 0;
+            endA = colsA > 0 ? fa.t_end : 0;
+            endB = colsB > 0 ? fb.t_end : 0;
+            r0A = colsA > 0 ? qlen - 1 - fa.q_end : 0;
+            r0B = colsB > 0 ? qlen - 1 - fb.q_end : 0;
+            rev_target = (colsA > 0 ? (unsigned)fa.score & 0xFFFFu : 0xFFFFu) | ((colsB > 0 ? (unsigned)fb.score & 0xFFFFu : 0xFFFFu) << 16);
+        }
+        int ncols = colsA > colsB ? colsA : colsB;
+        ncols = max(ncols, __shfl_xor(ncols, 16));
+        ncols = max(ncols, __shfl_xor(ncols, 32));
+        ncols = __builtin_amdgcn_readfirstlane(ncols);
+        const int nsteps = ncols + GROUP - 1;
+        int mincols = colsA < colsB ? colsA : colsB;
+        mincols = min(mincols, __shfl_xor(mincols, 16));
+        mincols = min(mincols, __shfl_xor(mincols, 32));
+        mincols = __builtin_amdgcn_readfirstlane(mincols);
+
+        unsigned long long bestA = 0, bestB = 0;
+
+        uint2 *scr = nullptr;
+        unsigned scr_grp = 0;
+        if (MULTI) {
+            scr = L.scratch + (size_t)((job.shape >> 8) * WAVES + wave) * GROUPS_PER_WAVE * 2 * L.scratch_cols;
+            scr_grp = (unsigned)grp * 2u * L.scratch_cols;
+        }
+
+        for (int tile = 0; tile < n_tiles; ++tile) {
+            const int tile_base = tile * T::ROWS;
+            if (MULTI && !resident) {
+                __syncthreads();
+                build_profile<R, REV>(lds, q, cb, qlen, tile_base, L.mat, L.alphabet, prof);
+                __syncthreads();
+            }
+            const unsigned char *const lds_tile = MULTI && resident ? lds + (uint32_t)tile * tile_bytes : lds;
+            const uint2 *scr_in = MULTI ? scr + (size_t)((tile + 1) & 1) * L.scratch_cols : nullptr;
+            uint2 *scr_out = MULTI ? scr + (size_t)(tile & 1) * L.scratch_cols : nullptr;
+            const bool has_above = MULTI && tile > 0;
+            const bool has_below = MULTI && tile + 1 < n_tiles;
+
+            unsigned Hp[R], E[R], aux[R];
+#pragma unroll
+            for (int r = 0; r < R; ++r) { Hp[r] = 0; E[r] = 0; aux[r] = 0; }
+            if (REV) {
+#pragma unroll
+                for (int r = 0; r < R; ++r) {
+                    const int rg = tile_base + g * R + r;
+                    aux[r] = (rg >= r0A ? 0xFFFFu : 0u) | (rg >= r0B ? 0xFFFF0000u : 0u);
+                }
+            }
+            unsigned vmax = 0, bestcol = 0xFFFFFFFFu;
+            unsigned rev_rowA = 0, rev_rowB = 0;
+            unsigned Hup_prev = 0;
+            unsigned out_H = 0, out_F = 0;
+
+            auto letters4 = [&](const uint8_t *p, int end, int k) -> unsigned {
+                if (!REV) return reinterpret_cast<const unsigned *>(p)[k];
+                int o = end - 3 - 4 * k;
+                o = o < -3 ? -3 : o;
+                unsigned w;
+                __builtin_memcpy(&w, p + o, 4);
+                return w;
+            };
+            unsigned wA = letters4(pA, endA, 0), wB = letters4(pB, endB, 0);
+            unsigned wA_next = letters4(pA, endA, 1), wB_next = letters4(pB, endB, 1);
+            uint2 bnd = make_uint2(0, 0), bnd_next = make_uint2(0, 0);
+            auto boundary16 = [&](int m) -> uint2 {
+                const int last = ncols - 1 < 0 ? 0 : ncols - 1;
+                return scr_in[scr_grp + (unsigned)min(16 * m + g - (m > 0 ? 1 : 0), last)];
+            };
+            if (has_above) {
+                bnd = boundary16(0);
+                bnd_next = boundary16(1);
+            }
+
+            constexpr int ND = (R + 1) / 2;
+            unsigned pav_next[PF ? ND : 1], pbv_next[PF ? ND : 1];
+            auto load_rows = [&](unsigned letters, unsigned *pav, unsigned *pbv) {
+                const unsigned a = letters & 0xFFu, b = (letters >> 8) & 0xFFu;
+                const uint4 *rowA = reinterpret_cast<const uint4 *>(lds_tile + a * T::ROW_STRIDE + g * T::LANE_STRIDE);
+                const uint4 *rowB = reinterpret_cast<const uint4 *>(lds_tile + b * T::ROW_STRIDE + g * T::LANE_STRIDE);
+#pragma unroll
+                for (int k = 0; k < ND / 4; ++k) {
+                    const uint4 pa = rowA[k], pb = rowB[k];
+                    pav[4 * k] = pa.x; pav[4 * k + 1] = pa.y; pav[4 * k + 2] = pa.z; pav[4 * k + 3] = pa.w;
+                    pbv[4 * k] = pb.x; pbv[4 * k + 1] = pb.y; pbv[4 * k + 2] = pb.z; pbv[4 * k + 3] = pb.w;
+                }
+                if constexpr (ND % 4 >= 2) {
+                    const uint2 pa = *reinterpret_cast<const uint2 *>(rowA + ND / 4);
+                    const uint2 pb = *reinterpret_cast<const uint2 *>(rowB + ND / 4);
+                    pav[(ND / 4) * 4] = pa.x; pav[(ND / 4) * 4 + 1] = pa.y;
+                    pbv[(ND / 4) * 4] = pb.x; pbv[(ND / 4) * 4 + 1] = pb.y;
+                }
+                if constexpr (ND % 2 == 1) {
+                    pav[ND - 1] = reinterpret_cast<const unsigned *>(rowA)[ND - 1];
+                    pbv[ND - 1] = reinterpret_cast<const unsigned *>(rowB)[ND - 1];
+                }
+            };
+            unsigned let = pad_letter * 0x101u;
+            constexpr bool LETTER_BLOCKS = MULTI || REV || R >= 7;
+            constexpr bool LETTER_QUEUE = !MULTI && R < 7;
+            unsigned long long lq = 0;
+            auto letter_block = [&](int k) {
+                if (!LETTER_BLOCKS) return;
+                unsigned a = wA, b = wB;
+                if (4 * k + 4 > mincols) {
+                    const unsigned pad4 = pad_letter * 0x01010101u;
+                    const int na = min(max(colsA - 4 * k, 0), 4), nb = min(max(colsB - 4 * k, 0), 4);
+                    const unsigned ma = REV ? ~(unsigned)(0xFFFFFFFFull >> (8 * na)) : (unsigned)((1ull << (8 * na)) - 1ull);
+                    const unsigned mb = REV ? ~(unsigned)(0xFFFFFFFFull >> (8 * nb)) : (unsigned)((1ull << (8 * nb)) - 1ull);
+                    a = bfi(ma, a, pad4);
+                    b = bfi(mb, b, pad4);
+                }
+                const unsigned lo = __builtin_amdgcn_perm(b, a, REV ? 0x06020703u : 0x05010400u);
+                const unsigned hi = __builtin_amdgcn_perm(b, a, REV ? 0x04000501u : 0x07030602u);
+                lq = ((unsigned long long)hi << 32) | lo;
+            };
+            auto head_letters = [&](int c, int j) -> unsigned {
+                if (LETTER_BLOCKS && LETTER_QUEUE) { const unsigned v = (unsigned)lq; lq >>= 16; return v; }
+                if (LETTER_BLOCKS) return (unsigned)(lq >> (16 * j));
+                const unsigned sh = (unsigned)(REV ? 3 - j : j) * 8u;
+                const unsigned la0 = __builtin_amdgcn_ubfe(wA, sh, 8u);
+                const unsigned lb0 = __builtin_amdgcn_ubfe(wB, sh, 8u);
+                return (c < colsA ? la0 : pad_letter) | ((c < colsB ? lb0 : pad_letter) << 8);
+            };
+            letter_block(0);
+            let = from_lane_above(head_letters(0, 0), let);
+            if (PF) load_rows(let, pav_next, pbv_next);
+
+            for (int s0 = -1; s0 < nsteps; s0 += 4) {
+            if (MULTI && s0 > 0 && ((s0 + 1) & 15) == 0) {
+                bnd = bnd_next;
+                if (has_above) bnd_next = boundary16(((s0 + 1) >> 4) + 1);
+            }
+            const int jn = min(4, nsteps - s0);
+#pragma nounroll
+            for (int j = s0 < 0 ? 1 : 0; j < jn; ++j) {
+                const int s = s0 + j;
+                if (has_below && s >= GROUP) {
+                    if (g == GROUP - 1) (scr_out + (s - GROUP))[scr_grp] = make_uint2(out_H, out_F);
+                }
+                const unsigned Hup = MULTI ? from_lane_above(bnd.x, out_H) : from_lane_above_or_zero(out_H);
+                unsigned f = MULTI ? from_lane_above(bnd.y, out_F) : from_lane_above_or_zero(out_F);
+                if (MULTI) {
+                    bnd.x = __builtin_amdgcn_update_dpp(bnd.x, bnd.x, 0x12F, 0xF, 0xF, false);
+                    bnd.y = __builtin_amdgcn_update_dpp(bnd.y, bnd.y, 0x12F, 0xF, 0xF, false);
+                }
+                unsigned pav[ND], pbv[ND];
+                if (PF) {
+#pragma unroll
+                    for (int k = 0; k < ND; ++k) { pav[k] = pav_next[k]; pbv[k] = pbv_next[k]; }
+                } else {
+                    load_rows(let, pav, pbv);
+                }
+
+                unsigned hd = Hup_prev;
+                Hup_prev = Hup;
+                unsigned cmax = 0;
+                unsigned pre[R], es[R];
+#pragma unroll
+                for (int r = 0; r < R; ++r) {
+                    unsigned P = __builtin_amdgcn_perm(pbv[r / 2], pav[r / 2], (r & 1) ? 0x07060302u : 0x05040100u);
+                    if (REV) P = __builtin_amdgcn_bitop3_b32(aux[r], P, NEG2, 0xCA);
+                    if constexpr (HALF) {
+                        pre[r] = h_add(r == 0 ? hd : Hp[r - 1], P);
+                        es[r] = h_sub(E[r], ge2);
+                    } else {
+                        pre[r] = pk_max_s(pk_add_sat(r == 0 ? hd : Hp[r - 1], P), E[r]);
+                        es[r] = pk_sub_sat_u(E[r], ge2);
+                    }
+                }
+                let = from_lane_above(head_letters(s + 1, j), let);
+                if (PF) load_rows(let, pav_next, pbv_next);
+#pragma unroll
+                for (int r = 0; r < R; ++r) {
+                    unsigned h;
+                    if constexpr (HALF) {
+                        h = h_max3(pre[r], E[r], f);
+                        const unsigned fs = h_sub(f, ge2);
+                        const unsigned t = h_sub(h, go2);
+                        cmax = r == 0 ? h : h_max(cmax, h);
+                        f = h_max3(fs, t, 0u);
+                        E[r] = h_max3(es[r], t, 0u);
+                    } else {
+                        h = pk_max_s(pre[r], f);
+                        const unsigned fs = pk_sub_sat_u(f, ge2);
+                        const unsigned t = pk_sub_sat_u(h, go2);
+                        cmax = pk_max_u(cmax, h);
+                        f = pk_max_u(fs, t);
+                        E[r] = pk_max_u(es[r], t);
+                    }
+                    SW_KEEP_IN_ROW(E[r]);
+                    Hp[r] = h;
+                }
+                out_H = Hp[R - 1];
+                out_F = f;
+
+                const int col = s - g;
+
+                const unsigned nm = pk_max_u(vmax, cmax);
+                if (nm != vmax) {
+                    const unsigned diff = nm ^ vmax;
+                    if (!REV) {
+                        const unsigned mask = ((diff & 0xFFFFu) ? 0xFFFFu : 0u) | ((diff >> 16) ? 0xFFFF0000u : 0u);
+                        bestcol = bfi(mask, ((unsigned)col & 0xFFFFu) * 0x10001u, bestcol);
+#pragma unroll
+                        for (int r = 0; r < R; ++r) aux[r] = bfi(mask, Hp[r], aux[r]);
+                    } else {
+                        const unsigned x = nm ^ rev_target;
+                        const bool hitA = (diff & 0xFFFFu) && !(x & 0xFFFFu), hitB = (diff >> 16) && !(x >> 16);
+                        if (hitA | hitB) {
+                            asm volatile("" ::: "memory");
+                            unsigned ra = 0, rb = 0;
+#pragma unroll
+                            for (int r = R - 1; r >= 0; --r) {
+                                if ((Hp[r] & 0xFFFFu) == (rev_target & 0xFFFFu)) ra = (unsigned)r;
+                                if ((Hp[r] >> 16) == (rev_target >> 16)) rb = (unsigned)r;
+                            }
+                            if (hitA) { bestcol = (bestcol & 0xFFFF0000u) | ((unsigned)col & 0xFFFFu); rev_rowA = ra; }
+                            if (hitB) { bestcol = (bestcol & 0xFFFFu) | ((unsigned)col << 16); rev_rowB = rb; }
+                        }
+                    }
+                    vmax = nm;
+                }
+            }
+            {
+                wA = wA_next; wB = wB_next;
+                const int k = ((s0 + 1) >> 2) + 2;
+                wA_next = letters4(pA, endA, k); wB_next = letters4(pB, endB, k);
+                letter_block(k - 1);
+            }
+            }
+            if (has_below && ncols > 0 && g == GROUP - 1) (scr_out + (ncols - 1))[scr_grp] = make_uint2(out_H, out_F);
+
+            unsigned rowA_first = rev_rowA, rowB_first = rev_rowB;
+            unsigned sA = vmax & 0xFFFFu, sB = vmax >> 16;
+            if (!REV) {
+#pragma unroll
+                for (int r = R - 1; r >= 0; --r) {
+                    if ((aux[r] & 0xFFFFu) == sA) rowA_first = (unsigned)r;
+                    if ((aux[r] >> 16) == sB) rowB_first = (unsigned)r;
+                }
+            } else {
+                sA = sA == (rev_target & 0xFFFFu) ? sA : 0u;
+                sB = sB == (rev_target >> 16) ? sB : 0u;
+            }
+            const unsigned rgA = (unsigned)(tile_base + g * R) + rowA_first;
+            const unsigned rgB = (unsigned)(tile_base + g * R) + rowB_first;
+            unsigned long long keyA = sA ? ((unsigned long long)sA << 32) | ((0xFFFFu - (bestcol & 0xFFFFu)) << 16) | (0xFFFFu - rgA) : 0ull;
+            unsigned long long keyB = sB ? ((unsigned long long)sB << 32) | ((0xFFFFu - (bestcol >> 16)) << 16) | (0xFFFFu - rgB) : 0ull;
+#pragma unroll
+            for (int m = 1; m < GROUP; m <<= 1) {
+                const unsigned long long oa = __shfl_xor(keyA, m), ob = __shfl_xor(keyB, m);
+                keyA = oa > keyA ? oa : keyA;
+                keyB = ob > keyB ? ob : keyB;
+            }
+            bestA = keyA > bestA ? keyA : bestA;
+            bestB = keyB > bestB ? keyB : bestB;
+        }
+
+        if (g == 0) {
+#pragma unroll
+            for (int half = 0; half < 2; ++half) {
+                const bool valid = half ? vB : vA;
+                if (!valid) continue;
+                const unsigned long long key = half ? bestB : bestA;
+                const uint32_t h = half ? hB : hA;
+                const bool marked = HALF && (unsigned)(key >> 32) > (unsigned)h_bits(SW_HALF_LIMIT);
+                const int score = HALF ? (marked ? SW_HALF_MARK : h_value((unsigned)(key >> 32))) : (int)(key >> 32);
+                const int col = 0xFFFF - (int)((key >> 16) & 0xFFFFu);
+                const int row = 0xFFFF - (int)(key & 0xFFFFu);
+                mmgpu_sw_hit *o = L.out + L.hit_out[h];
+                if (!REV) {
+                    mmgpu_sw_hit res;
+                    res.score = score;
+                    res.q_end = score ? row : 0;
+                    res.t_end = score ? col : -1;
+                    res.q_start = -1;
+                    res.t_start = -1;
+                    res.word = (score + qbias >= 255) ? 1 : 0;
+                    *o = res;
+                    if (marked) *half_flag = 1;
+                } else {
+                    const int end = half ? endB : endA;
+                    const int cols = half ? colsB : colsA;
+                    if (cols > 0) {
+                        o->t_start = (score == o->score) ? end - col : -2;
+                        o->q_start = (score == o->score) ? qlen - 1 - row : -2;
+                    }
+                }
+            }
+        }
+    }
+}
+
+template <int R, bool MULTI, bool BOTH>
+__device__ __forceinline__ void sw_passes(const SwLaunch &L, const SwJob &job) {
+    if constexpr (R <= SW_MAX_R) {
+        constexpr bool PF = MMGPU_SW_PREFETCH && !MULTI && (BOTH || R <= 24);
+        if (!(BOTH && L.rev_only)) sw_body<R, MULTI, false, PF>(L, job);
+        if constexpr (BOTH && !MULTI) {
+            __threadfence_block();
+            __syncthreads();
+            sw_body<R, MULTI, true, PF>(L, job);
+        }
+    }
+}
+
+#ifndef MMGPU_SW_WAVES_G0F
+#define MMGPU_SW_WAVES_G0F 4
+#endif
+#ifndef MMGPU_SW_WAVES_G0B
+#define MMGPU_SW_WAVES_G0B 2
+#endif
+#ifndef MMGPU_SW_WAVES_G1F
+#define MMGPU_SW_WAVES_G1F 3
+#endif
+#ifndef MMGPU_SW_WAVES_G1B
+#define MMGPU_SW_WAVES_G1B 2
+#endif
+
+}
+
+}
diff --git a/mmseqs2_amd/csrc/sw_half_kernel.hip b/mmseqs2_amd/csrc/sw_half_kernel.hip
--- /dev/null
+++ b/mmseqs2_amd/csrc/sw_half_kernel.hip
@@ -0,0 +1,87 @@
+#include "mmgpu_internal.h"
+#include "pf_device.h"
+#include "sw_body.h"
+
+namespace mmgpu {
+
+namespace {
+
+template <int R, bool BOTH>
+__device__ __forceinline__ void sw_half_passes(const SwLaunch &L, const SwJob &job) {
+    if constexpr (R <= SW_MAX_R) {
+        constexpr bool PF = MMGPU_SW_PREFETCH && (BOTH || R <= 24);
+        sw_body<R, false, false, PF, true, false>(L, job);
+        __threadfence_block();
+        __syncthreads();
+        if (sw_half_any_marked()) {
+            sw_body<R, false, false, PF, false, true>(L, job);
+            __threadfence_block();
+            __syncthreads();
+        }
+        if constexpr (BOTH) sw_body<R, false, true, PF>(L, job);
+    }
+}
+
+constexpr bool SW_HALF_FORWARD_ONLY[3] = {false, false, false};
+
+template <int G, bool BOTH>
+__global__ __launch_bounds__(WAVES * 64)
+__attribute__((amdgpu_waves_per_eu(G == 0 ? (BOTH ? MMGPU_SW_WAVES_G0B : MMGPU_SW_WAVES_G0F)
+                                           : (G == 1 ? (BOTH ? MMGPU_SW_WAVES_G1B : MMGPU_SW_WAVES_G1F) : SW_MIN_WAVES),
+                                   G == 1 && BOTH ? MMGPU_SW_WAVES_G1B : 8))) void sw_half_kernel(SwLaunch L) {
+    SwJob job = L.jobs[blockIdx.x];
+    if (L.q_hit_count) {
+        const uint32_t lim = job.query * L.hit_stride + L.q_hit_count[job.query];
+        job.hit_end = job.hit_end < lim ? job.hit_end : lim;
+        if (job.hit_end <= job.hit_begin) return;
+    }
+#define MMGPU_SW_SINGLE(R) case (R) - 1: sw_half_passes<R, BOTH>(L, job); break;
+    if constexpr (G == 0) {
+        switch (job.shape & 0xFFu) {
+            MMGPU_SW_SINGLE(1) MMGPU_SW_SINGLE(2) MMGPU_SW_SINGLE(3) MMGPU_SW_SINGLE(4) MMGPU_SW_SINGLE(5) MMGPU_SW_SINGLE(6)
+            MMGPU_SW_SINGLE(7) MMGPU_SW_SINGLE(8) MMGPU_SW_SINGLE(9) MMGPU_SW_SINGLE(10) MMGPU_SW_SINGLE(11) MMGPU_SW_SINGLE(12)
+            default: break;
+        }
+    } else if constexpr (G == 1) {
+        switch (job.shape & 0xFFu) {
+            MMGPU_SW_SINGLE(13) MMGPU_SW_SINGLE(14) MMGPU_SW_SINGLE(15) MMGPU_SW_SINGLE(16) MMGPU_SW_SINGLE(17) MMGPU_SW_SINGLE(18)
+            MMGPU_SW_SINGLE(19) MMGPU_SW_SINGLE(20) MMGPU_SW_SINGLE(21) MMGPU_SW_SINGLE(22) MMGPU_SW_SINGLE(23) MMGPU_SW_SINGLE(24)
+            default: break;
+        }
+    } else {
+        switch (job.shape & 0xFFu) {
+            MMGPU_SW_SINGLE(25) MMGPU_SW_SINGLE(26) MMGPU_SW_SINGLE(27) MMGPU_SW_SINGLE(28) MMGPU_SW_SINGLE(29) MMGPU_SW_SINGLE(30)
+            MMGPU_SW_SINGLE(31) MMGPU_SW_SINGLE(32)
+            default: break;
+        }
+    }
+#undef MMGPU_SW_SINGLE
+}
+
+#ifdef MMGPU_SW_HALF_AUDIT_FORWARD
+template __global__ void sw_half_kernel<0, false>(SwLaunch);
+template __global__ void sw_half_kernel<1, false>(SwLaunch);
+template __global__ void sw_half_kernel<2, false>(SwLaunch);
+#endif
+
+}
+
+bool launch_sw_half(const SwLaunch &L, int group, size_t lds_bytes, bool both_passes, hipStream_t stream) {
+    if (group < 0 || group > 2 || (group == 2 && SW_GROUPS != 4)) return false;
+    if (!both_passes && !SW_HALF_FORWARD_ONLY[group]) return false;
+    dim3 grid(L.n_jobs), block(WAVES * 64);
+    const size_t lds = lds_bytes + SW_LDS_HEADER;
+    switch (group) {
+        case 0: hipLaunchKernelGGL((sw_half_kernel<0, true>), grid, block, lds, stream, L); break;
+        case 1: hipLaunchKernelGGL((sw_half_kernel<1, true>), grid, block, lds, stream, L); break;
+        default: hipLaunchKernelGGL((sw_half_kernel<2, true>), grid, block, lds, stream, L); break;
+    }
+    return true;
+}
+
+void warm_sw_half() {
+    hipFuncAttributes a;
+    (void)hipFuncGetAttributes(&a, reinterpret_cast<const void *>(&sw_half_kernel<0, true>));
+}
+
+}
diff --git a/mmseqs2_amd/csrc/sw_kernel.hip b/mmseqs2_amd/csrc/sw_kernel.hip
--- a/mmseqs2_amd/csrc/sw_kernel.hip
+++ b/mmseqs2_amd/csrc/sw_kernel.hip
@@ -1,494 +1,11 @@
 #include "mmgpu_internal.h"
 #include "pf_device.h"
+#include "sw_body.h"
 
 namespace mmgpu {
 
 namespace {
 
-constexpr int GROUP = 16;
-constexpr int WAVES = 4;
-constexpr int GROUPS_PER_WAVE = 64 / GROUP;
-constexpr int HITS_PER_WAVE = 2 * GROUPS_PER_WAVE;
-constexpr unsigned NEG2 = 0x80008000u;
-
-typedef short s16x2 __attribute__((ext_vector_type(2)));
-typedef unsigned short u16x2 __attribute__((ext_vector_type(2)));
-
-__device__ __forceinline__ unsigned pk_add_sat(unsigned a, unsigned b) {
-    return __builtin_bit_cast(unsigned, __builtin_elementwise_add_sat(__builtin_bit_cast(s16x2, a),
-                                                                      __builtin_bit_cast(s16x2, b)));
-}
-__device__ __forceinline__ unsigned pk_max_s(unsigned a, unsigned b) {
-    return __builtin_bit_cast(unsigned, __builtin_elementwise_max(__builtin_bit_cast(s16x2, a),
-                                                                  __builtin_bit_cast(s16x2, b)));
-}
-__device__ __forceinline__ unsigned pk_max_u(unsigned a, unsigned b) {
-    return __builtin_bit_cast(unsigned, __builtin_elementwise_max(__builtin_bit_cast(u16x2, a),
-                                                                  __builtin_bit_cast(u16x2, b)));
-}
-__device__ __forceinline__ unsigned pk_sub_sat_u(unsigned a, unsigned b) {
-    return __builtin_bit_cast(unsigned, __builtin_elementwise_sub_sat(__builtin_bit_cast(u16x2, a),
-                                                                      __builtin_bit_cast(u16x2, b)));
-}
-__device__ __forceinline__ unsigned bfi(unsigned mask, unsigned a, unsigned b) {
-    return (a & mask) | (b & ~mask);
-}
-__device__ __forceinline__ unsigned from_lane_above(unsigned head, unsigned v) {
-    return __builtin_amdgcn_update_dpp(head, v, 0x111 , 0xF, 0xF, false);
-}
-__device__ __forceinline__ unsigned from_lane_above_or_zero(unsigned v) {
-    return __builtin_amdgcn_update_dpp(0u, v, 0x111 , 0xF, 0xF, true);
-}
-
-#ifndef MMGPU_SW_PREFETCH
-#define MMGPU_SW_PREFETCH 1
-#endif
-#define SW_KEEP_IN_ROW(x) asm volatile("" : "+v"(x))
-
-template <int R>
-struct Tile {
-    static constexpr int ROWS = GROUP * R;
-    static constexpr int LANE_STRIDE = lane_stride_bytes(R);
-    static constexpr int ROW_STRIDE = GROUP * LANE_STRIDE;
-};
-static_assert(GROUP == 16, "sw_profile_bytes and sw_tiles (mmgpu_internal.h) assume 16-lane groups");
-
-template <int R, bool REV>
-__device__ __forceinline__ void build_profile(unsigned char *lds, const uint8_t *q, const int8_t *cb, int qlen,
-                                              int tile_base, const int8_t *mat, int alphabet, const int8_t *prof) {
-    using T = Tile<R>;
-    const int total = (alphabet + 1) * T::ROWS;
-    for (int idx = threadIdx.x; idx < total; idx += blockDim.x) {
-        const int letter = idx / T::ROWS;
-        const int row = idx - letter * T::ROWS;
-        const int rg = tile_base + row;
-        short v = (short)-32768;
-        if (letter < alphabet && rg < qlen) {
-            const int qi = REV ? (qlen - 1 - rg) : rg;
-            v = prof ? (short)prof[letter * qlen + qi] : (short)((int)mat[letter * alphabet + q[qi]] + (int)cb[qi]);
-        }
-        const int lane = row / R, r = row - lane * R;
-        *reinterpret_cast<short *>(lds + letter * T::ROW_STRIDE + lane * T::LANE_STRIDE + r * 2) = v;
-    }
-}
-
-__device__ __forceinline__ bool sw_rev_wanted(const SwLaunch &L, uint32_t slot, int min_start) {
-    const mmgpu_sw_hit &f = L.out[slot];
-    const int s = f.score;
-    if (L.rev_mode == 2) return s > 0 && L.rev_force[slot] != 0;
-    return s > 0 && s >= min_start && !(L.rev_mode == 1 && f.word != 0);
-}
-
-constexpr int SW_REV_JOB_HITS = 1024;
-static_assert(SW_REV_JOB_HITS == SW_REV_JOB_MAX, "host and kernel disagree on the reverse job size");
-static_assert(SW_LDS_HEADER == SW_REV_JOB_HITS * 2 + 64, "the header holds the live hits and the scheduling words");
-
-template <int R, bool MULTI, bool REV, bool PF>
-__device__ __forceinline__ void sw_body(const SwLaunch &L, const SwJob job) {
-    using T = Tile<R>;
-    extern __shared__ __attribute__((aligned(16))) unsigned char lds_all[];
-    uint16_t *live = reinterpret_cast<uint16_t *>(lds_all);
-    uint32_t *live_wave = reinterpret_cast<uint32_t *>(lds_all + SW_REV_JOB_HITS * 2);
-    uint32_t *next_chunk = reinterpret_cast<uint32_t *>(lds_all + SW_REV_JOB_HITS * 2 + 16);
-    unsigned char *lds = lds_all + SW_LDS_HEADER;
-    if (MULTI) __builtin_amdgcn_s_setprio(3);
-    const int lane = threadIdx.x & 63;
-    const int wave = __builtin_amdgcn_readfirstlane(threadIdx.x >> 6);
-    const int g = lane & (GROUP - 1);
-    const int grp = lane / GROUP;
-
-    const uint32_t qbeg = L.q_off[job.query];
-    const int qlen = (int)(L.q_off[job.query + 1] - qbeg);
-    const uint8_t *q = L.q_res + qbeg;
-    const int8_t *cb = L.q_cb + qbeg;
-    const int qbias = L.q_bias[job.query];
-    const int8_t *prof = nullptr;
-    if (L.q_prof_off) {
-        const uint32_t po = L.q_prof_off[job.query];
-        if (po != 0xFFFFFFFFu) prof = L.q_prof + po;
-    }
-    const int n_tiles = MULTI ? (int)sw_tiles((uint32_t)qlen, R) : 1;
-    const uint32_t tile_bytes = sw_profile_bytes(R, L.alphabet);
-    const bool resident = MULTI && sw_multi_resident((uint32_t)n_tiles, R, L.alphabet, L.resident_lds);
-    const bool dynamic = !MULTI || resident;
-    auto build_all_tiles = [&]() {
-        for (int tile = 0; tile < n_tiles; ++tile)
-            build_profile<R, REV>(lds + (uint32_t)tile * tile_bytes, q, cb, qlen, tile * T::ROWS, L.mat, L.alphabet, prof);
-        __syncthreads();
-    };
-
-    const unsigned go2 = (unsigned)L.gap_open * 0x10001u;
-    const unsigned ge2 = (unsigned)L.gap_extend * 0x10001u;
-    const unsigned pad_letter = (unsigned)L.alphabet;
-
-    if (threadIdx.x == 0) *next_chunk = 0;
-    if (!MULTI && !REV) {
-        build_profile<R, REV>(lds, q, cb, qlen, 0, L.mat, L.alphabet, prof);
-        __syncthreads();
-    }
-    if (MULTI && !REV && resident) build_all_tiles();
-
-    uint32_t n_hits = job.hit_end - job.hit_begin;
-    if (REV) {
-        const int min_start = L.q_minstart[job.query];
-        uint32_t total = 0;
-        for (uint32_t base = 0; base < n_hits; base += WAVES * 64) {
-            const uint32_t idx = base + threadIdx.x;
-            bool pass = false;
-            if (idx < n_hits) pass = sw_rev_wanted(L, L.hit_out[job.hit_begin + idx], min_start);
-            const unsigned long long bal = __ballot(pass);
-            if (lane == 0) live_wave[wave] = (uint32_t)__popcll(bal);
-            __syncthreads();
-            uint32_t before = 0, round_total = 0;
-#pragma unroll
-            for (int w = 0; w < WAVES; ++w) {
-                const uint32_t c = live_wave[w];
-                before += w < wave ? c : 0u;
-                round_total += c;
-            }
-            if (pass) live[total + before + (uint32_t)__popcll(bal & ((1ull << lane) - 1ull))] = (uint16_t)idx;
-            total += round_total;
-            __syncthreads();
-        }
-        n_hits = total;
-        if (n_hits == 0) return;
-        if (!MULTI) {
-            build_profile<R, REV>(lds, q, cb, qlen, 0, L.mat, L.alphabet, prof);
-            __syncthreads();
-        }
-        if (MULTI && resident) build_all_tiles();
-    }
-    const uint32_t n_iter = (n_hits + WAVES * HITS_PER_WAVE - 1) / (WAVES * HITS_PER_WAVE);
-
-    for (uint32_t it = 0; dynamic || it < n_iter; ++it) {
-        uint32_t chunk = it * WAVES + wave;
-        if (dynamic) {
-            if (lane == 0) chunk = atomicAdd(next_chunk, 1u);
-            chunk = __builtin_amdgcn_readfirstlane(chunk);
-        }
-        const uint32_t slot0 = chunk * HITS_PER_WAVE;
-        if (dynamic && slot0 >= n_hits) break;
-
-        const uint32_t sA = slot0 + grp * 2, sB = sA + 1;
-        const bool vA = sA < n_hits, vB = sB < n_hits;
-        const uint32_t hA = job.hit_begin + (REV ? (uint32_t)live[vA ? sA : 0] : sA);
-        const uint32_t hB = job.hit_begin + (REV ? (uint32_t)live[vB ? sB : 0] : sB);
-        const uint32_t tA = vA ? L.hit_target[hA] : 0u, tB = vB ? L.hit_target[hB] : 0u;
-        const uint8_t *pA = L.t_res + (size_t)L.t_off4[tA] * 4;
-        const uint8_t *pB = L.t_res + (size_t)L.t_off4[tB] * 4;
-        int colsA = vA ? (int)L.t_len[tA] : 0, colsB = vB ? (int)L.t_len[tB] : 0;
-        int r0A = 0, r0B = 0;
-        int endA = 0, endB = 0;
-        unsigned rev_target = 0xFFFFFFFFu;
-        if (REV) {
-            mmgpu_sw_hit fa, fb;
-            fa.score = 0; fa.q_end = 0; fa.t_end = 0;
-            fb = fa;
-            if (vA) fa = L.out[L.hit_out[hA]];
-            if (vB) fb = L.out[L.hit_out[hB]];
-            colsA = vA ? fa.t_end + 1 : 0;
-            colsB = vB ? fb.t_end + 1 : 0;
-            endA = colsA > 0 ? fa.t_end : 0;
-            endB = colsB > 0 ? fb.t_end : 0;
-            r0A = colsA > 0 ? qlen - 1 - fa.q_end : 0;
-            r0B = colsB > 0 ? qlen - 1 - fb.q_end : 0;
-            rev_target = (colsA > 0 ? (unsigned)fa.score & 0xFFFFu : 0xFFFFu) | ((colsB > 0 ? (unsigned)fb.score & 0xFFFFu : 0xFFFFu) << 16);
-        }
-        int ncols = colsA > colsB ? colsA : colsB;
-        ncols = max(ncols, __shfl_xor(ncols, 16));
-        ncols = max(ncols, __shfl_xor(ncols, 32));
-        ncols = __builtin_amdgcn_readfirstlane(ncols);
-        const int nsteps = ncols + GROUP - 1;
-        int mincols = colsA < colsB ? colsA : colsB;
-        mincols = min(mincols, __shfl_xor(mincols, 16));
-        mincols = min(mincols, __shfl_xor(mincols, 32));
-        mincols = __builtin_amdgcn_readfirstlane(mincols);
-
-        unsigned long long bestA = 0, bestB = 0;
-
-        uint2 *scr = nullptr;
-        unsigned scr_grp = 0;
-        if (MULTI) {
-            scr = L.scratch + (size_t)((job.shape >> 8) * WAVES + wave) * GROUPS_PER_WAVE * 2 * L.scratch_cols;
-            scr_grp = (unsigned)grp * 2u * L.scratch_cols;
-        }
-
-        for (int tile = 0; tile < n_tiles; ++tile) {
-            const int tile_base = tile * T::ROWS;
-            if (MULTI && !resident) {
-                __syncthreads();
-                build_profile<R, REV>(lds, q, cb, qlen, tile_base, L.mat, L.alphabet, prof);
-                __syncthreads();
-            }
-            const unsigned char *const lds_tile = MULTI && resident ? lds + (uint32_t)tile * tile_bytes : lds;
-            const uint2 *scr_in = MULTI ? scr + (size_t)((tile + 1) & 1) * L.scratch_cols : nullptr;
-            uint2 *scr_out = MULTI ? scr + (size_t)(tile & 1) * L.scratch_cols : nullptr;
-            const bool has_above = MULTI && tile > 0;
-            const bool has_below = MULTI && tile + 1 < n_tiles;
-
-            unsigned Hp[R], E[R], aux[R];
-#pragma unroll
-            for (int r = 0; r < R; ++r) { Hp[r] = 0; E[r] = 0; aux[r] = 0; }
-            if (REV) {
-#pragma unroll
-                for (int r = 0; r < R; ++r) {
-                    const int rg = tile_base + g * R + r;
-                    aux[r] = (rg >= r0A ? 0xFFFFu : 0u) | (rg >= r0B ? 0xFFFF0000u : 0u);
-                }
-            }
-            unsigned vmax = 0, bestcol = 0xFFFFFFFFu;
-            unsigned rev_rowA = 0, rev_rowB = 0;
-            unsigned Hup_prev = 0;
-            unsigned out_H = 0, out_F = 0;
-
-            auto letters4 = [&](const uint8_t *p, int end, int k) -> unsigned {
-                if (!REV) return reinterpret_cast<const unsigned *>(p)[k];
-                int o = end - 3 - 4 * k;
-                o = o < -3 ? -3 : o;
-                unsigned w;
-                __builtin_memcpy(&w, p + o, 4);
-                return w;
-            };
-            unsigned wA = letters4(pA, endA, 0), wB = letters4(pB, endB, 0);
-            unsigned wA_next = letters4(pA, endA, 1), wB_next = letters4(pB, endB, 1);
-            uint2 bnd = make_uint2(0, 0), bnd_next = make_uint2(0, 0);
-            auto boundary16 = [&](int m) -> uint2 {
-                const int last = ncols - 1 < 0 ? 0 : ncols - 1;
-                return scr_in[scr_grp + (unsigned)min(16 * m + g - (m > 0 ? 1 : 0), last)];
-            };
-            if (has_above) {
-                bnd = boundary16(0);
-                bnd_next = boundary16(1);
-            }
-
-            constexpr int ND = (R + 1) / 2;
-            unsigned pav_next[PF ? ND : 1], pbv_next[PF ? ND : 1];
-            auto load_rows = [&](unsigned letters, unsigned *pav, unsigned *pbv) {
-                const unsigned a = letters & 0xFFu, b = (letters >> 8) & 0xFFu;
-                const uint4 *rowA = reinterpret_cast<const uint4 *>(lds_tile + a * T::ROW_STRIDE + g * T::LANE_STRIDE);
-                const uint4 *rowB = reinterpret_cast<const uint4 *>(lds_tile + b * T::ROW_STRIDE + g * T::LANE_STRIDE);
-#pragma unroll
-                for (int k = 0; k < ND / 4; ++k) {
-                    const uint4 pa = rowA[k], pb = rowB[k];
-                    pav[4 * k] = pa.x; pav[4 * k + 1] = pa.y; pav[4 * k + 2] = pa.z; pav[4 * k + 3] = pa.w;
-                    pbv[4 * k] = pb.x; pbv[4 * k + 1] = pb.y; pbv[4 * k + 2] = pb.z; pbv[4 * k + 3] = pb.w;
-                }
-                if constexpr (ND % 4 >= 2) {
-                    const uint2 pa = *reinterpret_cast<const uint2 *>(rowA + ND / 4);
-                    const uint2 pb = *reinterpret_cast<const uint2 *>(rowB + ND / 4);
-                    pav[(ND / 4) * 4] = pa.x; pav[(ND / 4) * 4 + 1] = pa.y;
-                    pbv[(ND / 4) * 4] = pb.x; pbv[(ND / 4) * 4 + 1] = pb.y;
-                }
-                if constexpr (ND % 2 == 1) {
-                    pav[ND - 1] = reinterpret_cast<const unsigned *>(rowA)[ND - 1];
-                    pbv[ND - 1] = reinterpret_cast<const unsigned *>(rowB)[ND - 1];
-                }
-            };
-            unsigned let = pad_letter * 0x101u;
-            constexpr bool LETTER_BLOCKS = MULTI || REV || R >= 7;
-            constexpr bool LETTER_QUEUE = !MULTI && R < 7;
-            unsigned long long lq = 0;
-            auto letter_block = [&](int k) {
-                if (!LETTER_BLOCKS) return;
-                unsigned a = wA, b = wB;
-                if (4 * k + 4 > mincols) {
-                    const unsigned pad4 = pad_letter * 0x01010101u;
-                    const int na = min(max(colsA - 4 * k, 0), 4), nb = min(max(colsB - 4 * k, 0), 4);
-                    const unsigned ma = REV ? ~(unsigned)(0xFFFFFFFFull >> (8 * na)) : (unsigned)((1ull << (8 * na)) - 1ull);
-                    const unsigned mb = REV ? ~(unsigned)(0xFFFFFFFFull >> (8 * nb)) : (unsigned)((1ull << (8 * nb)) - 1ull);
-                    a = bfi(ma, a, pad4);
-                    b = bfi(mb, b, pad4);
-                }
-                const unsigned lo = __builtin_amdgcn_perm(b, a, REV ? 0x06020703u : 0x05010400u);
-                const unsigned hi = __builtin_amdgcn_perm(b, a, REV ? 0x04000501u : 0x07030602u);
-                lq = ((unsigned long long)hi << 32) | lo;
-            };
-            auto head_letters = [&](int c, int j) -> unsigned {
-                if (LETTER_BLOCKS && LETTER_QUEUE) { const unsigned v = (unsigned)lq; lq >>= 16; return v; }
-                if (LETTER_BLOCKS) return (unsigned)(lq >> (16 * j));
-                const unsigned sh = (unsigned)(REV ? 3 - j : j) * 8u;
-                const unsigned la0 = __builtin_amdgcn_ubfe(wA, sh, 8u);
-                const unsigned lb0 = __builtin_amdgcn_ubfe(wB, sh, 8u);
-                return (c < colsA ? la0 : pad_letter) | ((c < colsB ? lb0 : pad_letter) << 8);
-            };
-            letter_block(0);
-            let = from_lane_above(head_letters(0, 0), let);
-            if (PF) load_rows(let, pav_next, pbv_next);
-
-            for (int s0 = -1; s0 < nsteps; s0 += 4) {
-            if (MULTI && s0 > 0 && ((s0 + 1) & 15) == 0) {
-                bnd = bnd_next;
-                if (has_above) bnd_next = boundary16(((s0 + 1) >> 4) + 1);
-            }
-            const int jn = min(4, nsteps - s0);
-#pragma nounroll
-            for (int j = s0 < 0 ? 1 : 0; j < jn; ++j) {
-                const int s = s0 + j;
-                if (has_below && s >= GROUP) {
-                    if (g == GROUP - 1) (scr_out + (s - GROUP))[scr_grp] = make_uint2(out_H, out_F);
-                }
-                const unsigned Hup = MULTI ? from_lane_above(bnd.x, out_H) : from_lane_above_or_zero(out_H);
-                unsigned f = MULTI ? from_lane_above(bnd.y, out_F) : from_lane_above_or_zero(out_F);
-                if (MULTI) {
-                    bnd.x = __builtin_amdgcn_update_dpp(bnd.x, bnd.x, 0x12F, 0xF, 0xF, false);
-                    bnd.y = __builtin_amdgcn_update_dpp(bnd.y, bnd.y, 0x12F, 0xF, 0xF, false);
-                }
-                unsigned pav[ND], pbv[ND];
-                if (PF) {
-#pragma unroll
-                    for (int k = 0; k < ND; ++k) { pav[k] = pav_next[k]; pbv[k] = pbv_next[k]; }
-                } else {
-                    load_rows(let, pav, pbv);
-                }
-
-                unsigned hd = Hup_prev;
-                Hup_prev = Hup;
-                unsigned cmax = 0;
-                unsigned pre[R], es[R];
-#pragma unroll
-                for (int r = 0; r < R; ++r) {
-                    unsigned P = __builtin_amdgcn_perm(pbv[r / 2], pav[r / 2], (r & 1) ? 0x07060302u : 0x05040100u);
-                    if (REV) P = __builtin_amdgcn_bitop3_b32(aux[r], P, NEG2, 0xCA);
-                    pre[r] = pk_max_s(pk_add_sat(r == 0 ? hd : Hp[r - 1], P), E[r]);
-                    es[r] = pk_sub_sat_u(E[r], ge2);
-                }
-                let = from_lane_above(head_letters(s + 1, j), let);
-                if (PF) load_rows(let, pav_next, pbv_next);
-#pragma unroll
-                for (int r = 0; r < R; ++r) {
-                    const unsigned h = pk_max_s(pre[r], f);
-                    const unsigned fs = pk_sub_sat_u(f, ge2);
-                    const unsigned t = pk_sub_sat_u(h, go2);
-                    cmax = pk_max_u(cmax, h);
-                    f = pk_max_u(fs, t);
-                    E[r] = pk_max_u(es[r], t);
-                    SW_KEEP_IN_ROW(E[r]);
-                    Hp[r] = h;
-                }
-                out_H = Hp[R - 1];
-                out_F = f;
-
-                const int col = s - g;
-
-                const unsigned nm = pk_max_u(vmax, cmax);
-                if (nm != vmax) {
-                    const unsigned diff = nm ^ vmax;
-                    if (!REV) {
-                        const unsigned mask = ((diff & 0xFFFFu) ? 0xFFFFu : 0u) | ((diff >> 16) ? 0xFFFF0000u : 0u);
-                        bestcol = bfi(mask, ((unsigned)col & 0xFFFFu) * 0x10001u, bestcol);
-#pragma unroll
-                        for (int r = 0; r < R; ++r) aux[r] = bfi(mask, Hp[r], aux[r]);
-                    } else {
-                        const unsigned x = nm ^ rev_target;
-                        const bool hitA = (diff & 0xFFFFu) && !(x & 0xFFFFu), hitB = (diff >> 16) && !(x >> 16);
-                        if (hitA | hitB) {
-                            asm volatile("" ::: "memory");
-                            unsigned ra = 0, rb = 0;
-#pragma unroll
-                            for (int r = R - 1; r >= 0; --r) {
-                                if ((Hp[r] & 0xFFFFu) == (rev_target & 0xFFFFu)) ra = (unsigned)r;
-                                if ((Hp[r] >> 16) == (rev_target >> 16)) rb = (unsigned)r;
-                            }
-                            if (hitA) { bestcol = (bestcol & 0xFFFF0000u) | ((unsigned)col & 0xFFFFu); rev_rowA = ra; }
-                            if (hitB) { bestcol = (bestcol & 0xFFFFu) | ((unsigned)col << 16); rev_rowB = rb; }
-                        }
-                    }
-                    vmax = nm;
-                }
-            }
-            {
-                wA = wA_next; wB = wB_next;
-                const int k = ((s0 + 1) >> 2) + 2;
-                wA_next = letters4(pA, endA, k); wB_next = letters4(pB, endB, k);
-                letter_block(k - 1);
-            }
-            }
-            if (has_below && ncols > 0 && g == GROUP - 1) (scr_out + (ncols - 1))[scr_grp] = make_uint2(out_H, out_F);
-
-            unsigned rowA_first = rev_rowA, rowB_first = rev_rowB;
-            unsigned sA = vmax & 0xFFFFu, sB = vmax >> 16;
-            if (!REV) {
-#pragma unroll
-                for (int r = R - 1; r >= 0; --r) {
-                    if ((aux[r] & 0xFFFFu) == sA) rowA_first = (unsigned)r;
-                    if ((aux[r] >> 16) == sB) rowB_first = (unsigned)r;
-                }
-            } else {
-                sA = sA == (rev_target & 0xFFFFu) ? sA : 0u;
-                sB = sB == (rev_target >> 16) ? sB : 0u;
-            }
-            const unsigned rgA = (unsigned)(tile_base + g * R) + rowA_first;
-            const unsigned rgB = (unsigned)(tile_base + g * R) + rowB_first;
-            unsigned long long keyA = sA ? ((unsigned long long)sA << 32) | ((0xFFFFu - (bestcol & 0xFFFFu)) << 16) | (0xFFFFu - rgA) : 0ull;
-            unsigned long long keyB = sB ? ((unsigned long long)sB << 32) | ((0xFFFFu - (bestcol >> 16)) << 16) | (0xFFFFu - rgB) : 0ull;
-#pragma unroll
-            for (int m = 1; m < GROUP; m <<= 1) {
-                const unsigned long long oa = __shfl_xor(keyA, m), ob = __shfl_xor(keyB, m);
-                keyA = oa > keyA ? oa : keyA;
-                keyB = ob > keyB ? ob : keyB;
-            }
-            bestA = keyA > bestA ? keyA : bestA;
-            bestB = keyB > bestB ? keyB : bestB;
-        }
-
-        if (g == 0) {
-#pragma unroll
-            for (int half = 0; half < 2; ++half) {
-                const bool valid = half ? vB : vA;
-                if (!valid) continue;
-                const unsigned long long key = half ? bestB : bestA;
-                const uint32_t h = half ? hB : hA;
-                const int score = (int)(key >> 32);
-                const int col = 0xFFFF - (int)((key >> 16) & 0xFFFFu);
-                const int row = 0xFFFF - (int)(key & 0xFFFFu);
-                mmgpu_sw_hit *o = L.out + L.hit_out[h];
-                if (!REV) {
-                    mmgpu_sw_hit res;
-                    res.score = score;
-                    res.q_end = score ? row : 0;
-                    res.t_end = score ? col : -1;
-                    res.q_start = -1;
-                    res.t_start = -1;
-                    res.word = (score + qbias >= 255) ? 1 : 0;
-                    *o = res;
-                } else {
-                    const int end = half ? endB : endA;
-                    const int cols = half ? colsB : colsA;
-                    if (cols > 0) {
-                        o->t_start = (score == o->score) ? end - col : -2;
-                        o->q_start = (score == o->score) ? qlen - 1 - row : -2;
-                    }
-                }
-            }
-        }
-    }
-}
-
-template <int R, bool MULTI, bool BOTH>
-__device__ __forceinline__ void sw_passes(const SwLaunch &L, const SwJob &job) {
-    if constexpr (R <= SW_MAX_R) {
-        constexpr bool PF = MMGPU_SW_PREFETCH && !MULTI && (BOTH || R <= 24);
-        if (!(BOTH && L.rev_only)) sw_body<R, MULTI, false, PF>(L, job);
-        if constexpr (BOTH && !MULTI) {
-            __threadfence_block();
-            __syncthreads();
-            sw_body<R, MULTI, true, PF>(L, job);
-        }
-    }
-}
-
-#ifndef MMGPU_SW_WAVES_G0F
-#define MMGPU_SW_WAVES_G0F 4
-#endif
-#ifndef MMGPU_SW_WAVES_G0B
-#define MMGPU_SW_WAVES_G0B 2
-#endif
-#ifndef MMGPU_SW_WAVES_G1F
-#define MMGPU_SW_WAVES_G1F 3
-#endif
-#ifndef MMGPU_SW_WAVES_G1B
-#define MMGPU_SW_WAVES_G1B 2
-#endif
 #define MMGPU_SW_MULTI_ALL                                                                                                          \
     MMGPU_SW_MULTI(8) MMGPU_SW_MULTI(9) MMGPU_SW_MULTI(10) MMGPU_SW_MULTI(11) MMGPU_SW_MULTI(12) MMGPU_SW_MULTI(13) MMGPU_SW_MULTI(14) \
     MMGPU_SW_MULTI(15) MMGPU_SW_MULTI(16) MMGPU_SW_MULTI(17) MMGPU_SW_MULTI(18) MMGPU_SW_MULTI(19) MMGPU_SW_MULTI(20) MMGPU_SW_MULTI(21) \
@@ -687,9 +204,15 @@
     return R <= 12 ? 0 : (R <= 24 ? 1 : 2);
 }
 
+static bool sw_half_eligible(const SwLaunch &L) {
+    return MMGPU_SW_HALF && !L.rev_only && L.gap_open >= 0 && L.gap_open <= SW_HALF_MAX_GAP && L.gap_extend >= 0 &&
+           L.gap_extend <= SW_HALF_MAX_GAP;
+}
+
 hipError_t launch_sw(const SwLaunch &L, int group, size_t lds_bytes, bool both_passes, hipStream_t stream) {
     static_assert(GROUP == 16, "the shape codes assume 16-lane groups");
     if (L.n_jobs == 0) return hipSuccess;
+    if (sw_half_eligible(L) && launch_sw_half(L, group, lds_bytes, both_passes, stream)) return hipGetLastError();
     dim3 grid(L.n_jobs), block(WAVES * 64);
     const size_t lds = lds_bytes + SW_LDS_HEADER;
     switch (group * 2 + (both_passes ? 1 : 0)) {
@@ -709,6 +232,7 @@
 void warm_sw() {
     hipFuncAttributes a;
     (void)hipFuncGetAttributes(&a, reinterpret_cast<const void *>(&sw_rev_multi_kernel));
-}
-
-}
+    if (MMGPU_SW_HALF) warm_sw_half();
+}
+
+}
```

After: 4939 (median of 6 runs). +5.7%, better.
